# tenpy/tenpy

Hardware: AMD Instinct MI355X
Metric: DMRG sweep time (s) + GS energy err, Heisenberg L=100 chi=2048 (lower is better)
Workload: dtype f64

## Files before the change

include/tenpy_amd.h:

```cpp
#ifndef TENPY_AMD_H
#define TENPY_AMD_H
#include <stdint.h>
#ifdef __cplusplus
extern "C" {
#endif

#define TPA_F64 0
#define TPA_C128 1

#define TPA_E_BADARG (-1)
#define TPA_E_NOCONV (-2)
#define TPA_E_NAN (-3)
#define TPA_E_NOMEM (-4)
#define TPA_E_RANKCAP (-5)

int tpa_version(void);
int tpa_device_info(char *name, int name_len, int *n_cu, int64_t *hbm_bytes);
const char *tpa_last_error(void);

int tpa_gemm_chain(int dtype, int cfg, const int64_t *tasks_dev, const int64_t *links_dev,
                   const int32_t *tiles_dev, int n_tiles, const void *Abase, const void *Bbase,
                   void *Cbase, void *stream);

int tpa_herk_tile_shape(int dtype, int *bt);
int tpa_herk_chain(int dtype, const int64_t *tasks_dev, const int64_t *links_dev, const int32_t *tiles_dev, int n_tiles,
                   const void *Abase, const void *Bbase, const double *wvec_dev, void *Cbase, void *stream);

#define TPA_RED_SCRATCH 4096
int tpa_axpy(int dtype, int64_t n, double alpha_re, double alpha_im, const void *x_dev,
             void *y_dev, void *stream);
int tpa_scal(int dtype, int64_t n, double alpha_re, double alpha_im, void *x_dev, void *stream);
int tpa_dot(int dtype, int64_t n, const void *x_dev, const void *y_dev, int do_conj,
            double *out_dev, double *scratch_dev, void *stream);
int tpa_nrm2sq(int dtype, int64_t n, const void *x_dev, double *out_dev, double *scratch_dev,
               void *stream);
int tpa_lanczos_update(int dtype, int64_t n, void *w_dev, double alpha_re, double alpha_im,
                       const void *v1_dev, double beta_re, double beta_im, const void *v0_dev,
                       double *out_dev, double *scratch_dev, void *stream);
int tpa_lanczos_step(int dtype, int64_t n, void *w_dev, const void *v1_dev, const void *v0_dev,
                     const double *bsq_prev_dev, double *ab_out_dev, double *scratch_dev, void *stream);

#define TPA_PROJECT_MAX 64
#define TPA_PROJECT_WORK (2 * 1024 * (TPA_PROJECT_MAX + 1))
int tpa_project_out(int dtype, int64_t n, const void *basis_dev, int m, int64_t stride, const void *src_dev, void *dst_dev,
                    double *coeff_dev, double *nrm2_out_dev, double *work_dev, void *stream);

typedef int (*tpa_lanczos_callback)(int step, double alpha, double beta_sq, void *user);
typedef int (*tpa_collective_callback)(int which, void *user);
int tpa_lanczos_set_collective(tpa_collective_callback cb, void *user);
int tpa_lanczos_run(int dtype, int64_t n, const int64_t *ops, int n_ops, void *const *bufs, int n_bufs,
                    void *krylov_dev, const void *psi0_dev, int N_max, double cutoff, int has_shift, double E_shift,
                    double *scalars_dev, double *scratch_dev, tpa_lanczos_callback cb, void *user,
                    int time_gemms, double *info, void *stream);
int tpa_lanczos_run_ex(int dtype, int64_t n, const int64_t *ops, int n_ops, void *const *bufs, int n_bufs,
                       void *krylov_dev, const void *psi0_dev, int N_max, double cutoff, int has_shift, double E_shift,
                       double *scalars_dev, double *scratch_dev, tpa_lanczos_callback cb, void *user,
                       int time_gemms, double *info, int flags, double *project_work_dev, void *stream);
int tpa_krylov_combine(int dtype, int64_t n, const void *krylov_dev, int N, const double *coeff, void *out_dev,
                       double *red_out_dev, double *scratch_dev, double *norm_host, void *stream);
int tpa_krylov_combine_z(int basis_dtype, int64_t n, const void *krylov_dev, int N, const double *coeff, double scale,
                         void *out_dev, double *red_out_dev, double *scratch_dev, double *norm_host, void *stream);

#define TPA_COPY_MAXDIM 6
int tpa_copy_batch(int dtype, const int64_t *jobs_dev, int n_jobs, int64_t max_job_elems,
                   const void *src_base, void *dst_base, void *stream);
int tpa_lincomb_batch(int dtype, const int64_t *jobs_dev, int n_jobs, const int64_t *terms_dev, int64_t max_job_elems,
                      const void *src_base, void *dst_base, void *stream);
#define TPA_MPO_APPLY_MAXD 16
int tpa_mpo_apply_batch(int dtype, const int64_t *jobs_dev, int n_jobs, const int64_t *terms_dev, const void *coeff_dev, int max_d,
                        int64_t max_job_elems, const void *src_base, void *dst_base, void *stream);
int tpa_mpo_entry_apply_batch(int dtype, const int64_t *jobs_dev, int n_jobs, const int64_t *rows_dev, const int64_t *terms_dev,
                              int64_t max_job_cols, const void *src_base, void *dst_base, void *stream);
int tpa_scale_axis_batch(int dtype, const int64_t *jobs_dev, int n_jobs, int64_t max_job_elems,
                         void *x_base, const void *s_dev, int s_is_complex, void *stream);
int tpa_fill_zero(void *dst_dev, int64_t n_bytes, void *stream);
int tpa_tri_lower_batch(int dtype, const int64_t *jobs_dev, int n_jobs, int64_t max_job_elems, void *g_base, void *stream);
int tpa_gather_axis_batch(int dtype, const int64_t *jobs_dev, int n_jobs, int64_t max_job_elems,
                          const int64_t *idx_dev, const void *src_base, void *dst_base, void *stream);
int tpa_axis_sqnorm_batch(int dtype, const int64_t *jobs_dev, const int32_t *rows_dev, int n_rows,
                          const void *x_base, double *out_dev, void *stream);
int tpa_convert(int from_dtype, int to_dtype, int64_t n, const void *src_dev, void *dst_dev, int conj,
                void *stream);
int tpa_gemm_tile_shape(int dtype, int cfg, int *bm, int *bn);
int tpa_gemm_set_variant(int v);

int64_t tpa_svd_worksize(int dtype, const int64_t *jobs_host, int n_jobs);
int tpa_svd_batch(int dtype, const int64_t *jobs_host, int n_jobs, const void *a_base,
                  void *u_base, double *s_dev, void *vh_base, void *work_dev, int64_t work_bytes,
                  int max_sweeps, double tol, int *sweeps_done, void *stream);

int tpa_svd_theta(int dtype, int side, const int64_t *blocks, int n_blocks, int64_t a_numel, const void *a_arena,
                  const void *basis_arena, void *u_arena, int64_t u_numel, void *v_arena, int64_t v_numel, double *s_host,
                  double e_tol, int lowdin_basis, int clean_iterations, double clean_floor, int alg_warm, int alg_restore,
                  int max_sweeps, double tol, int *sweeps_done, double *info, void *stream);
int tpa_svd_theta_store(int dtype, const int64_t *blocks, const int64_t *ksig, int n_blocks, const void *u_arena, const void *v_arena,
                        void *basis_r, void *basis_l, void *stream);

int tpa_svd_set_algorithm(int pairwise);
int tpa_svd_dyn_stats(int64_t *out, int reset);
int64_t tpa_svd_call_log(int64_t *out, int64_t max_rows, int reset);
int tpa_svd_set_rank_cap(int cap);

int tpa_qr_batch(int dtype, const int64_t *jobs_host, int n_jobs, const void *a_base, void *q_base,
                 void *r_base, void *stream);
int tpa_qr_set_algorithm(int v);

int64_t tpa_eigh_worksize(int dtype, const int64_t *jobs_host, int n_jobs);
int tpa_eigh_batch(int dtype, const int64_t *jobs_host, int n_jobs, const void *a_base,
                   double *w_dev, void *v_base, void *work_dev, int64_t work_bytes, int max_sweeps,
                   double tol, int *sweeps_done, void *stream);
int tpa_eigh_set_direct(int on);
int tpa_eigh_last_direct(void);
int tpa_eigh_from_svd(int dtype, const int64_t *jobs_host, int n_jobs, const void *u_base, const double *s_dev,
                      const void *vh_base, double *lam_dev, double *err_dev, void *stream);

int tpa_plan_tensordot(const int64_t *a_qdata, int64_t na, int ra, const int64_t *b_qdata,
                       int64_t nb, int rb, int ncontr, const int64_t *contr_nblocks,
                       int64_t *res_qdata, int64_t *res_a_first, int64_t *res_b_first,
                       int64_t cap_res, int64_t *n_res, int64_t *gemm, int64_t cap_gemm,
                       int64_t *n_gemm);

#ifdef __cplusplus
}
#endif
#endif
```

tenpy_amd/_lib.py:

```python
import ctypes
import os

import numpy as np

from . import _build

F64, C128 = 0, 1
E_BADARG, E_NOCONV, E_NAN, E_NOMEM, E_RANKCAP = -1, -2, -3, -4, -5
PROJECT_MAX = 64
PROJECT_WORK = 2 * 1024 * (PROJECT_MAX + 1)
MPO_APPLY_MAXD = 16

_lib = None

_i64p = ctypes.POINTER(ctypes.c_int64)
_vp = ctypes.c_void_p
LANCZOS_CALLBACK = ctypes.CFUNCTYPE(ctypes.c_int, ctypes.c_int, ctypes.c_double, ctypes.c_double, ctypes.c_void_p)
COLLECTIVE_CALLBACK = ctypes.CFUNCTYPE(ctypes.c_int, ctypes.c_int, ctypes.c_void_p)
_SIGS = {
    "tpa_version": (ctypes.c_int, []),
    "tpa_last_error": (ctypes.c_char_p, []),
    "tpa_device_info": (ctypes.c_int, [ctypes.c_char_p, ctypes.c_int, ctypes.POINTER(ctypes.c_int), _i64p]),
    "tpa_gemm_tile_shape": (ctypes.c_int, [ctypes.c_int, ctypes.c_int, ctypes.POINTER(ctypes.c_int), ctypes.POINTER(ctypes.c_int)]),
    "tpa_gemm_set_variant": (ctypes.c_int, [ctypes.c_int]),
    "tpa_gemm_chain": (ctypes.c_int, [ctypes.c_int, ctypes.c_int, _vp, _vp, _vp, ctypes.c_int, _vp, _vp, _vp, _vp]),
    "tpa_herk_tile_shape": (ctypes.c_int, [ctypes.c_int, ctypes.POINTER(ctypes.c_int)]),
    "tpa_herk_chain": (ctypes.c_int, [ctypes.c_int, _vp, _vp, _vp, ctypes.c_int, _vp, _vp, _vp, _vp, _vp]),
    "tpa_axpy": (ctypes.c_int, [ctypes.c_int, ctypes.c_int64, ctypes.c_double, ctypes.c_double, _vp, _vp, _vp]),
    "tpa_scal": (ctypes.c_int, [ctypes.c_int, ctypes.c_int64, ctypes.c_double, ctypes.c_double, _vp, _vp]),
    "tpa_dot": (ctypes.c_int, [ctypes.c_int, ctypes.c_int64, _vp, _vp, ctypes.c_int, _vp, _vp, _vp]),
    "tpa_nrm2sq": (ctypes.c_int, [ctypes.c_int, ctypes.c_int64, _vp, _vp, _vp, _vp]),
    "tpa_lanczos_update": (ctypes.c_int, [ctypes.c_int, ctypes.c_int64, _vp, ctypes.c_double, ctypes.c_double, _vp,
                                          ctypes.c_double, ctypes.c_double, _vp, _vp, _vp, _vp]),
    "tpa_lanczos_step": (ctypes.c_int, [ctypes.c_int, ctypes.c_int64, _vp, _vp, _vp, _vp, _vp, _vp, _vp]),
    "tpa_lanczos_run": (ctypes.c_int, [ctypes.c_int, ctypes.c_int64, _vp, ctypes.c_int, _vp, ctypes.c_int, _vp, _vp, ctypes.c_int,
                                       ctypes.c_double, ctypes.c_int, ctypes.c_double, _vp, _vp, _vp, _vp, ctypes.c_int, _vp, _vp]),
    "tpa_lanczos_run_ex": (ctypes.c_int, [ctypes.c_int, ctypes.c_int64, _vp, ctypes.c_int, _vp, ctypes.c_int, _vp, _vp, ctypes.c_int,
                                          ctypes.c_double, ctypes.c_int, ctypes.c_double, _vp, _vp, _vp, _vp, ctypes.c_int, _vp,
                                          ctypes.c_int, _vp, _vp]),
    "tpa_project_out": (ctypes.c_int, [ctypes.c_int, ctypes.c_int64, _vp, ctypes.c_int, ctypes.c_int64, _vp, _vp, _vp, _vp, _vp, _vp]),
    "tpa_lanczos_set_collective": (ctypes.c_int, [COLLECTIVE_CALLBACK, _vp]),
    "tpa_krylov_combine": (ctypes.c_int, [ctypes.c_int, ctypes.c_int64, _vp, ctypes.c_int, _vp, _vp, _vp, _vp, _vp, _vp]),
    "tpa_krylov_combine_z": (ctypes.c_int, [ctypes.c_int, ctypes.c_int64, _vp, ctypes.c_int, _vp, ctypes.c_double, _vp, _vp, _vp, _vp, _vp]),
    "tpa_copy_batch": (ctypes.c_int, [ctypes.c_int, _vp, ctypes.c_int, ctypes.c_int64, _vp, _vp, _vp]),
    "tpa_lincomb_batch": (ctypes.c_int, [ctypes.c_int, _vp, ctypes.c_int, _vp, ctypes.c_int64, _vp, _vp, _vp]),
    "tpa_mpo_apply_batch": (ctypes.c_int, [ctypes.c_int, _vp, ctypes.c_int, _vp, _vp, ctypes.c_int, ctypes.c_int64, _vp, _vp, _vp]),
    "tpa_mpo_entry_apply_batch": (ctypes.c_int, [ctypes.c_int, _vp, ctypes.c_int, _vp, _vp, ctypes.c_int64, _vp, _vp, _vp]),
    "tpa_svd_dyn_stats": (ctypes.c_int, [_i64p, ctypes.c_int]),
    "tpa_tri_lower_batch": (ctypes.c_int, [ctypes.c_int, _vp, ctypes.c_int, ctypes.c_int64, _vp, _vp]),
    "tpa_scale_axis_batch": (ctypes.c_int, [ctypes.c_int, _vp, ctypes.c_int, ctypes.c_int64, _vp, _vp, ctypes.c_int, _vp]),
    "tpa_gather_axis_batch": (ctypes.c_int, [ctypes.c_int, _vp, ctypes.c_int, ctypes.c_int64, _vp, _vp, _vp, _vp]),
    "tpa_axis_sqnorm_batch": (ctypes.c_int, [ctypes.c_int, _vp, _vp, ctypes.c_int, _vp, _vp, _vp]),
    "tpa_convert": (ctypes.c_int, [ctypes.c_int, ctypes.c_int, ctypes.c_int64, _vp, _vp, ctypes.c_int, _vp]),
    "tpa_fill_zero": (ctypes.c_int, [_vp, ctypes.c_int64, _vp]),
    "tpa_svd_worksize": (ctypes.c_int64, [ctypes.c_int, _vp, ctypes.c_int]),
    "tpa_svd_batch": (ctypes.c_int, [ctypes.c_int, _vp, ctypes.c_int, _vp, _vp, _vp, _vp, _vp, ctypes.c_int64,
                                     ctypes.c_int, ctypes.c_double, ctypes.POINTER(ctypes.c_int), _vp]),
    "tpa_svd_set_algorithm": (ctypes.c_int, [ctypes.c_int]),
    "tpa_svd_theta": (ctypes.c_int, [ctypes.c_int, ctypes.c_int, _vp, ctypes.c_int, ctypes.c_int64, _vp, _vp, _vp, ctypes.c_int64, _vp, ctypes.c_int64,
                                     _vp, ctypes.c_double, ctypes.c_int, ctypes.c_int, ctypes.c_double, ctypes.c_int, ctypes.c_int, ctypes.c_int,
                                     ctypes.c_double, ctypes.POINTER(ctypes.c_int), _vp, _vp]),
    "tpa_svd_theta_store": (ctypes.c_int, [ctypes.c_int, _vp, _vp, ctypes.c_int, _vp, _vp, _vp, _vp, _vp]),
    "tpa_svd_set_rank_cap": (ctypes.c_int, [ctypes.c_int]),
    "tpa_svd_call_log": (ctypes.c_int64, [_i64p, ctypes.c_int64, ctypes.c_int]),
    "tpa_qr_batch": (ctypes.c_int, [ctypes.c_int, _vp, ctypes.c_int, _vp, _vp, _vp, _vp]),
    "tpa_qr_set_algorithm": (ctypes.c_int, [ctypes.c_int]),
    "tpa_eigh_worksize": (ctypes.c_int64, [ctypes.c_int, _vp, ctypes.c_int]),
    "tpa_eigh_batch": (ctypes.c_int, [ctypes.c_int, _vp, ctypes.c_int, _vp, _vp, _vp, _vp, ctypes.c_int64,
                                      ctypes.c_int, ctypes.c_double, ctypes.POINTER(ctypes.c_int), _vp]),
    "tpa_eigh_set_direct": (ctypes.c_int, [ctypes.c_int]),
    "tpa_eigh_last_direct": (ctypes.c_int, []),
    "tpa_eigh_from_svd": (ctypes.c_int, [ctypes.c_int, _vp, ctypes.c_int, _vp, _vp, _vp, _vp, _vp, _vp]),
    "tpa_plan_tensordot": (ctypes.c_int, [_vp, ctypes.c_int64, ctypes.c_int, _vp, ctypes.c_int64, ctypes.c_int,
                                          ctypes.c_int, _vp, _vp, _vp, _vp, ctypes.c_int64, _i64p, _vp,
                                          ctypes.c_int64, _i64p]),
}


class BackendError(RuntimeError):
    """The HIP extension is missing or a HIP runtime call failed."""


def load(build_if_missing=True):
    global _lib
    if _lib is not None:
        return _lib
    import torch
    path = _build.LIB_PATH
    alt = os.environ.get('TPA_LIB_PATH')
    if alt:
        if not os.path.exists(alt):
            raise BackendError("tenpy_amd: TPA_LIB_PATH=%s does not exist" % alt)
        path, build_if_missing = alt, False
    if not os.path.exists(path):
        if not build_if_missing:
            raise BackendError("tenpy_amd: %s not built; run `python -m tenpy_amd._build`" % path)
        _build.build()
    elif build_if_missing and os.path.exists(_build.HIPCC) and os.path.isdir(_build.CSRC) and not os.environ.get('TPA_NO_AUTOBUILD'):
        import fcntl
        try:
            with open(os.path.join(_build.OUT_DIR, '.build.lock'), 'w') as lock:
                fcntl.flock(lock, fcntl.LOCK_EX)
                try:
                    _build.build()
                finally:
                    fcntl.flock(lock, fcntl.LOCK_UN)
        except OSError:
            pass
    lib = ctypes.CDLL(path)
    for name, (res, args) in _SIGS.items():
        f = getattr(lib, name)
        f.restype = res
        f.argtypes = args
    _lib = lib
    return lib


def exported_symbols():
    return sorted(_SIGS)


def check(rc, what=""):
    if rc == 0:
        return
    msg = load().tpa_last_error()
    msg = msg.decode() if msg else ""
    if rc == E_BADARG:
        raise ValueError("tenpy_amd %s: %s" % (what, msg))
    if rc == E_NOCONV:
        raise np.linalg.LinAlgError("tenpy_amd %s: %s" % (what, msg))
    if rc == E_NAN:
        raise ValueError("tenpy_amd %s: NaN/Inf encountered: %s" % (what, msg))
    raise BackendError("tenpy_amd %s: HIP error %d: %s" % (what, rc, msg))


_gpu_ok = False


def require_gpu():
    global _gpu_ok
    if _gpu_ok:
        return
    import torch
    if not torch.cuda.is_available():
        raise BackendError("tenpy_amd: no GPU visible (torch.cuda.is_available() is False); "
                           "this backend has no CPU fallback")
    load()
    _gpu_ok = True
```

tenpy_amd/algorithms/mps_common.py:

```python
import numpy as np

from ..linalg import _device as dev
from ..linalg import np_conserved as npc

__all__ = ['TwoSiteH', 'OneSiteH', 'ZeroSiteH']


FUSED_HEFF = True
import os as _os
FACTORED_MATVEC = _os.environ.get('TPA_FACTORED_MATVEC', '1') != '0'
FACTORED_MIN_SECTOR = 200
BLOCK_APPLY = _os.environ.get('TPA_MPO_BLOCK_APPLY', '1') != '0'
from .._lib import MPO_APPLY_MAXD
ENTRY_APPLY = int(_os.environ.get('TPA_MPO_ENTRY_APPLY', '1'))

def _env_set_LP(env, i, LP):
    if hasattr(env, 'get_LP_age'):
        env.set_LP(i, LP, age=(env.get_LP_age(i - 1) or 0) + 1)
    else:
        env.set_LP(i, LP)


def _env_set_RP(env, i, RP):
    if hasattr(env, 'get_RP_age'):
        env.set_RP(i, RP, age=(env.get_RP_age(i + 1) or 0) + 1)
    else:
        env.set_RP(i, RP)


def _mpo_entries(W):
    ent = getattr(W, '_tpa_entries', False)
    if ent is False:
        if all(np.all(leg.get_block_sizes() == 1) for leg in W.legs) and W.stored_blocks > 0:
            vals = np.array([np.asarray(b).reshape(-1)[0] for b in W._data])
            ent = (np.array(W._qdata), vals)
        else:
            ent = None
        W._tpa_entries = ent
    return ent


def _mpo_blocks(W):
    blk = getattr(W, '_tpa_blocks', False)
    if blk is False:
        labels = list(W.get_leg_labels())
        blk = None
        if W.rank == 4 and 'wL' in labels and 'wR' in labels and W.stored_blocks > 0 and W.chinfo.qnumber > 0:
            phys = [a for a in range(4) if labels[a] not in ('wL', 'wR')]
            if all(np.all(W.get_leg(l).get_block_sizes() == 1) for l in ('wL', 'wR')) and \
                    all(int(np.max(W.legs[a].get_block_sizes())) <= MPO_APPLY_MAXD for a in phys):
                blk = (np.array(W._qdata), [np.array(b) for b in W._data])
        W._tpa_blocks = blk
    return blk


def _share_mpo_tables(W_new, W):
    W_new._tpa_entries = _mpo_entries(W)
    if W_new._tpa_entries is None and BLOCK_APPLY and dev.lib_provides('tpa_mpo_apply_batch'):
        W_new._tpa_blocks = _mpo_blocks(W)
    W_new._tpa_origin = W


def _mpo_coo(W):
    coo = getattr(W, '_tpa_coo', False)
    if coo is False and getattr(W, '_tpa_origin', None) is not None:
        coo = W._tpa_coo = _mpo_coo(W._tpa_origin)
    if coo is False:
        labels = list(W.get_leg_labels())
        coo = None
        if W.rank == 4 and 'wL' in labels and 'wR' in labels and W.stored_blocks > 0:
            idx, vals = [], []
            for q, b in zip(np.array(W._qdata).tolist(), W._data):
                b = np.array(b)
                nz = np.nonzero(b)
                idx.append(np.stack([nz[a] + int(W.legs[a].slices[q[a]]) for a in range(4)], axis=1))
                vals.append(b[nz])
            coo = (np.concatenate(idx).astype(np.int64).reshape(-1, 4), np.concatenate(vals))
        W._tpa_coo = coo
    return coo


def _pack_alpha(terms, alpha):
    alpha = np.asarray(alpha, dtype=np.complex128)
    terms[:, 2] = np.ascontiguousarray(alpha.real).view(np.int64)
    terms[:, 3] = np.ascontiguousarray(alpha.imag).view(np.int64)


def _lincomb_into(dst, src, jobs, terms, max_elems):
    if len(jobs) == 0:
        return
    L = dev.lib()
    terms_d = dev.table(terms)
    for s0 in range(0, len(jobs), 60000):
        jd = dev.table(jobs[s0:s0 + 60000])
        dev.check(L.tpa_lincomb_batch(dev.code(dst.dtype), jd.data_ptr(), len(jobs[s0:s0 + 60000]), terms_d.data_ptr(),
                                      int(max_elems), src._arena.data_ptr(), dst._arena.data_ptr(), dev.stream()), "lincomb")


def _rank_rows(q):
    uq, inv = np.unique(q, axis=0, return_inverse=True)
    order = np.lexsort(uq.T)
    rank_of = np.empty(len(order), dtype=np.int64)
    rank_of[order] = np.arange(len(order))
    return uq[order], rank_of[inv.reshape(-1)]


def _group_terms(dst):
    key = np.lexsort((np.arange(len(dst)), dst))
    d_sorted = dst[key]
    starts = np.nonzero(np.concatenate([[True], d_sorted[1:] != d_sorted[:-1]]))[0]
    return key, starts, np.diff(np.concatenate([starts, [len(key)]]))


from collections import OrderedDict as _OrderedDict
_heff_plans = _OrderedDict()


def _fused_heff(env_t, W, left):
    from ..linalg.charges import LegPipe
    ent = _mpo_entries(W)
    pl = 'p0' if left else 'p1'
    want_env = ['vR*', 'wR', 'vR'] if left else ['wL', 'vL', 'vL*']
    if ent is None or list(env_t.get_leg_labels()) != want_env or list(W.get_leg_labels()) != ['wL', 'wR', pl, pl + '*'] \
            or env_t.dtype != np.result_type(env_t.dtype, W.dtype) or env_t.stored_blocks == 0:
        return None
    wq, wv = ent
    w_axis_env = 1 if left else 0
    if not np.all(env_t.legs[w_axis_env].get_block_sizes() == 1):
        return None
    pkey = (left, env_t._struct_key(), env_t.dtype.str, id(ent), env_t.qtotal.tobytes(),
            tuple((l.charges.tobytes(), int(l.qconj)) for l in env_t.legs))
    plan = _heff_plans.get(pkey)
    if plan is not None and plan['ent'] is ent:
        try:
            _heff_plans.move_to_end(pkey)
        except KeyError:
            pass
        res = npc.Array(plan['legs'], env_t.dtype, plan['qtotal'], plan['labels'])
        res._adopt_blocks(plan['qdata'], plan['offsets'], dev.zeros(plan['total'], env_t.dtype), True)
        dev.check(dev.lib().tpa_lincomb_batch(dev.code(env_t.dtype), plan['jobs'].data_ptr(), plan['n_jobs'], plan['terms'].data_ptr(),
                                              plan['max_elems'], env_t._arena.data_ptr(), res._arena.data_ptr(), dev.stream()), "lincomb")
        return res, plan['pipe']
    eq = env_t._qdata
    shapes = env_t._block_shapes()
    if left:
        pipe = LegPipe([env_t.get_leg('vR*'), W.get_leg('p0')], qconj=+1)
        legs = [pipe, W.get_leg('wR'), pipe.conj()]
        labels = ['(vR*.p0)', 'wR', '(vR.p0*)']
    else:
        pipe = LegPipe([W.get_leg('p1'), env_t.get_leg('vL*')], qconj=-1)
        legs = [W.get_leg('wL'), pipe.conj(), pipe]
        labels = ['wL', '(p1*.vL)', '(p1.vL*)']
    qm = pipe.q_map
    n0, n1 = pipe.legs[0].block_number, pipe.legs[1].block_number
    row_of = np.full((n0, n1), -1, dtype=np.int64)
    row_of[qm[:, 3], qm[:, 4]] = np.arange(len(qm))
    psz = pipe.get_block_sizes()
    wc = wq[:, 0] if left else wq[:, 1]
    ie, iw = np.nonzero(eq[:, w_axis_env][:, None] == wc[None, :])
    if len(ie) == 0:
        return None
    if left:
        r_row = row_of[eq[ie, 0], wq[iw, 2]]
        c_row = row_of[eq[ie, 2], wq[iw, 3]]
        w_out = wq[iw, 1]
        rows, cols = shapes[ie, 0], shapes[ie, 2]
    else:
        r_row = row_of[wq[iw, 3], eq[ie, 1]]
        c_row = row_of[wq[iw, 2], eq[ie, 2]]
        w_out = wq[iw, 0]
        rows, cols = shapes[ie, 1], shapes[ie, 2]
    Qr, Qc = qm[r_row, 2], qm[c_row, 2]
    r0, c0 = qm[r_row, 0], qm[c_row, 0]
    bq = np.stack([Qr, w_out, Qc], axis=1) if left else np.stack([w_out, Qr, Qc], axis=1)
    ubq, blk = _rank_rows(bq)
    res = npc.Array(legs, env_t.dtype, env_t.chinfo.make_valid(env_t.qtotal + W.qtotal), labels)
    res._set_blocks(ubq, zero=True, qdata_sorted=True)
    ld = psz[Qc]
    dst_off = res._offsets[blk] + r0 * ld + c0
    perm, starts, counts = _group_terms(dst_off)
    jobs = np.zeros((len(starts), 8), dtype=np.int64)
    pf = perm[starts]
    jobs[:, 0], jobs[:, 1], jobs[:, 2], jobs[:, 3] = dst_off[pf], rows[pf], cols[pf], ld[pf]
    jobs[:, 4], jobs[:, 5] = starts, counts
    terms = np.zeros((len(perm), 4), dtype=np.int64)
    terms[:, 0] = env_t._offsets[ie[perm]]
    terms[:, 1] = shapes[ie[perm], 2]
    _pack_alpha(terms, wv[iw[perm]])
    _lincomb_into(res, env_t, jobs, terms, int(np.max(rows * cols)))
    if 0 < len(jobs) <= 60000:
        for arr in (res._qdata, res._offsets):
            arr.setflags(write=False)
        _heff_plans[pkey] = dict(ent=ent, legs=legs, labels=labels, qtotal=res.qtotal.copy(), qdata=res._qdata, offsets=res._offsets,
                                 total=int(res._arena.numel()), jobs=dev.table(jobs), terms=dev.table(terms), n_jobs=len(jobs),
                                 max_elems=int(np.max(rows * cols)), pipe=pipe)
        if len(_heff_plans) > 8192:
            _heff_plans.popitem(last=False)
    return res, pipe


def _reverse_columns(U):
    res = npc.Array(U.legs, U.dtype, U.qtotal, list(U._labels))
    res._set_blocks(U._qdata, zero=False, qdata_sorted=U._qdata_sorted)
    if U.stored_blocks == 0:
        return res
    shapes = U._block_shapes()
    m, k = shapes[:, 0], shapes[:, 1]
    blk = np.repeat(np.arange(len(k)), k)
    col = np.arange(len(blk)) - np.repeat(np.cumsum(k) - k, k)
    jobs = np.zeros((len(blk), 8), dtype=np.int64)
    jobs[:, 0] = res._offsets[blk] + col
    jobs[:, 1], jobs[:, 2], jobs[:, 3] = m[blk], 1, k[blk]
    jobs[:, 4], jobs[:, 5] = np.arange(len(blk)), 1
    terms = np.zeros((len(blk), 4), dtype=np.int64)
    terms[:, 0] = U._offsets[blk] + (k[blk] - 1 - col)
    terms[:, 1] = k[blk]
    terms[:, 2] = np.array([1.0]).view(np.int64)[0]
    _lincomb_into(res, U, jobs, terms, int(np.max(m)))
    return res


def _relabel_view(A, labels):
    perm = [A.get_leg_index(l) for l in labels]
    if perm == list(range(A.rank)):
        return A
    big = [a for a in range(A.rank) if not np.all(A.legs[a].get_block_sizes() == 1)]
    assert [a for a in perm if a in big] == big, "only legs with 1-wide blocks may be moved"
    B = A.copy(deep=False)
    B.legs = [A.legs[a] for a in perm]
    B._set_shape()
    B._labels = [A._labels[a] for a in perm]
    B._qdata = np.ascontiguousarray(A._qdata[:, perm])
    B._offsets = A._offsets.copy()
    B._qdata_sorted = False
    B._skey = None
    B.isort_qdata()
    return B


class _MpoStepPlan:

    @classmethod
    def get(cls, X, W, *args, W2=None, **kwargs):
        t1, t2 = cls._table(W), (None if W2 is None else cls._table(W2))
        key = (X._struct_key(), str(X.dtype), id(t1), None if t2 is None else id(t2), args,
               tuple(sorted(kwargs.items())), tuple(X.get_leg_labels()))
        plan = cls._cache.get(key)
        if plan is None or plan._tables_alive[0] is not t1 or plan._tables_alive[1] is not t2:
            if len(cls._cache) > 4096:
                cls._cache.clear()
            plan = cls._cache[key] = cls(X, W, *args, W2=W2, **kwargs)
            plan._tables_alive = (t1, t2)
        return plan

    @staticmethod
    def _match_blocks(X, keys, xa):
        xq = X._qdata
        match = xq[:, xa[0]][:, None] == keys[None, :, 0]
        for a, col in zip(xa[1:], (3, 5)):
            match &= xq[:, a][:, None] == keys[None, :, col]
        ib, ie = np.nonzero(match)
        oq = xq[ib].copy()
        for a, col in zip(xa, (1, 2, 4)):
            oq[:, a] = keys[ie, col]
        return ib, ie, oq

    def _set_output(self, X, W, W2, xa, w_out, p_out, p2_out, out_labels):
        self.dtype = np.result_type(X.dtype, W.dtype) if W2 is None else np.result_type(X.dtype, W.dtype, W2.dtype)
# ... 294 lines not shown
        self.x_key = X._struct_key()
        self.bytes = 8 * (2 if self.dtype.kind == 'c' else 1) * (self.total + int(np.sum(shapes_x[ib, 0] * post_x)))

    def _launch(self, X, res):
        dev.check(dev.lib().tpa_mpo_entry_apply_batch(dev.code(self.dtype), self.jobs_dev.data_ptr(), self.n_jobs, self.rows_dev.data_ptr(),
                                                      self.terms_dev.data_ptr(), self.max_cols, X._arena.data_ptr(), res._arena.data_ptr(),
                                                      dev.stream()), "mpo_entry_apply")

    def program_op(self, a_slot, c_slot):
        return [6, 0, self.jobs_dev.data_ptr(), self.rows_dev.data_ptr(), self.terms_dev.data_ptr(), self.n_jobs, a_slot, 0, c_slot,
                self.max_cols, 0, 0]


def _envs_wide(LP, RP):
    return not (bool(np.all(LP.get_leg('wR').get_block_sizes() == 1)) and bool(np.all(RP.get_leg('wL').get_block_sizes() == 1)))


def _envs_factorable(LP, RP):
    lp, rp = list(LP.get_leg_labels()), list(RP.get_leg_labels())
    return (sorted(lp) == sorted(['vR*', 'wR', 'vR']) and lp.index('vR*') < lp.index('vR') and
            sorted(rp) == sorted(['wL', 'vL', 'vL*']) and rp.index('vL') < rp.index('vL*') and
            (not _envs_wide(LP, RP) or _entry_route(LP.chinfo)))


def _env_form(A, labels):
    if list(A.get_leg_labels()) == list(labels):
        return A
    w = 'wR' if 'wR' in labels else 'wL'
    if np.all(A.get_leg(w).get_block_sizes() == 1):
        return _relabel_view(A, labels)
    return A.transpose(labels)


def _factored_plan_class(LP, RP, W, W2=None):
    if not _envs_factorable(LP, RP):
        return None
    cls = _mpo_plan_class(W, W2)
    if cls is not MpoEntryApplyPlan and _envs_wide(LP, RP):
        return None
    return cls


def factored_matvec_possible(LP, RP, W0, W1):
    w0, w1 = list(W0.get_leg_labels()), list(W1.get_leg_labels())
    return (_factored_plan_class(LP, RP, W0, W1) is not None and
            w0 in (['wL', 'wR', 'p0', 'p0*'], ['wL', 'wR', 'p', 'p*']) and w1 in (['wL', 'wR', 'p1', 'p1*'], ['wL', 'wR', 'p', 'p*']))


def _gemm_ops(plan, a_slot, b_slot, c_slot, bufs, scratch_name):
    sk = plan.sk
    if sk is None:
        return [[0, plan.cfg, plan.tasks_dev.data_ptr(), plan.links_dev.data_ptr(), plan.tiles_dev.data_ptr(), plan.n_tiles,
                 a_slot, b_slot, c_slot, 0, 0, 0]]
    bufs.append(dev.scratch(scratch_name, sk.total, plan.dtype))
    part = len(bufs) - 1
    return [[0, plan.cfg, sk.tasks_dev.data_ptr(), sk.links_dev.data_ptr(), sk.tiles_dev.data_ptr(), sk.n_tiles, a_slot, b_slot, part, 0, 0, 0],
            [1, 1, sk.jobs_dev.data_ptr(), sk.terms_dev.data_ptr(), 0, sk.n_jobs, part, 0, c_slot, sk.max_elems, 0, 0]]


_STEP_LR = ('wR', 'p0', 'wL', 'wR', 'p0', 'p0*')
_STEP_RL = ('wL', 'p1', 'wR', 'wL', 'p1', 'p1*')


def _mpo_step_lr(X, W0, W1=None, *, out_labels):
    two = {} if W1 is None else dict(W2=W1, x_p2='p1', p2_out='p1', p2_in='p1*')
    return _mpo_plan_class(W0, W1).get(X, W0, *_STEP_LR, tuple(out_labels), **two)


def _mpo_step_rl(X, W1, *, out_labels):
    return _mpo_plan_class(W1).get(X, W1, *_STEP_RL, tuple(out_labels))


def _factored_plans(LPf, RPf, theta, W0, W1=None, launch=False, old=None):
    keys = dict(key=theta._struct_key(), dtype=theta.dtype, lkey=LPf._struct_key(), rkey=RPf._struct_key())
    if old is not None and all(old[k] == v for k, v in keys.items()):
        return old, None, None
    p1, l_use, t_use = npc.plan_tensordot(LPf, theta, axes=['vR', 'vL'])
    fits = l_use is LPf and t_use is theta
    assert fits or not launch, "factored matvec step 1 must not need a transpose"
    if not fits or (p1.empty and not launch):
        return None, None, None
    T = T1 = p1.apply(LPf, theta, launch=launch)
    a = None
    if W0 is not None:
        a = _mpo_step_lr(T1, W0, W1, out_labels=('vR*', 'p0', 'wR', 'vR') if W1 is None else ('vR*', 'p0', 'p1', 'wR', 'vR'))
        if a.empty and not launch:
            return None, None, None
        T = a.apply(T1, launch=launch)
    p2, t_use, r_use = npc.plan_tensordot(T, RPf, axes=(['wR', 'vR'], ['wL', 'vL']))
    fits = t_use is T and r_use is RPf
    assert fits or not launch, "factored matvec step 2 must not need a transpose"
    if not fits or (p2.empty and not launch):
        return None, None, None
    return dict(keys, p1=p1, p2=p2, **{'a0' if W1 is None else 'a01': a}), T1, T


class _DeviceEffectiveH:

    def _file_program(self, theta, res, last):
        key = (theta._struct_key(), theta.dtype)
        self.__dict__['_program_out'] = None
        if res is not None and not (last.res_total == theta._arena.numel() and np.array_equal(last.res_qdata, theta._qdata)
                                    and np.array_equal(last.res_offsets, theta._offsets)):
            self.__dict__['_program_out'] = (key, last.res_qdata, last.res_offsets, last.res_total)
            res = None
        self.__dict__['_program'] = (key, res)
        return res

    def native_input(self, theta, max_pad=2):
        vec = theta
        for _ in range(max_pad + 1):
            prog = self.matvec_program(vec)
            if prog is not None:
                return vec, prog
            out = self.__dict__.get('_program_out')
            if out is None or out[0] != (vec._struct_key(), vec.dtype):
                return None
            _, qdata, offsets, total = out
            have = {tuple(r) for r in qdata.tolist()}
            if not all(tuple(r) in have for r in vec._qdata.tolist()):
                return None
            pad = npc.Array(vec.legs, vec.dtype, vec.qtotal, vec.get_leg_labels())
            pad._set_blocks(qdata, arena=dev.zeros(total, vec.dtype), qdata_sorted=True)
            if not np.array_equal(pad._offsets, offsets):
                return None
            npc._scatter_blocks(vec, pad, pad._arena)
            vec = pad
        return None


class TwoSiteH(_DeviceEffectiveH):
    length = 2
    acts_on = ['(vL.p0)', '(p1.vR)']

    def __init__(self, env, i0, combine=True, move_right=True, tensors=None, factored=None):
        if not combine:
            raise NotImplementedError("tenpy_amd.TwoSiteH (stand-alone driver): only combine=True")
        self.i0 = i0
        self.combine = combine
        self.move_right = move_right
        if tensors is not None:
            self.LP, self.RP, W0, W1 = tensors
            self.dtype = W0.dtype
        else:
            self.LP = env.get_LP(i0)
            self.RP = env.get_RP(i0 + 1)
            W0, W1 = env.H.get_W(i0), env.H.get_W(i0 + 1)
            self.dtype = env.H.dtype
        self.W0 = W0.replace_labels(['p', 'p*'], ['p0', 'p0*'])
        self.W1 = W1.replace_labels(['p', 'p*'], ['p1', 'p1*'])
        _share_mpo_tables(self.W0, W0)
        _share_mpo_tables(self.W1, W1)
        self._env = env
        self._LHeff = self._RHeff = None
        self._plans = None
        self._fplans = None
        if factored is None:
            want = FACTORED_MATVEC and int(np.max(self.LP.get_leg('vR').get_block_sizes())) >= FACTORED_MIN_SECTOR
        else:
            want = factored
        self.factored = bool(want) and self._factored_possible()
        if self.factored:
            from ..linalg.charges import LegPipe
            self._LPf = _env_form(self.LP, ['vR*', 'wR', 'vR'])
            self._RPf = _env_form(self.RP, ['wL', 'vL', 'vL*'])
            self.pipeL = LegPipe([self.LP.get_leg('vR*'), self.W0.get_leg('p0')], qconj=+1)
            self.pipeR = LegPipe([self.W1.get_leg('p1'), self.RP.get_leg('vL*')], qconj=-1)
            self._LHeff = self._RHeff = None
            self.acts_on = ['vL', 'p0', 'p1', 'vR']
        else:
            self.combine_Heff(self._env)
        self.N = self.pipeL.ind_len * self.pipeR.ind_len
        self.flops_per_matvec = None
        self.bytes_per_matvec = None

    def _factored_possible(self):
        return factored_matvec_possible(self.LP, self.RP, self.W0, self.W1)

    @property
    def LHeff(self):
        if self._LHeff is None:
            self._build_heff_lazily()
        return self._LHeff

    @LHeff.setter
    def LHeff(self, value):
        self._LHeff = value

    @property
    def RHeff(self):
        if self._RHeff is None:
            self._build_heff_lazily()
        return self._RHeff

    @RHeff.setter
    def RHeff(self, value):
        self._RHeff = value

    def _build_heff_lazily(self):
        pL, pR = self.pipeL, self.pipeR
        self.combine_Heff(self._env)
        pL.test_equal(self.pipeL)
        pR.test_equal(self.pipeR)
        self.pipeL, self.pipeR = pL, pR

    def combine_Heff(self, env=None):
        cache = getattr(env, '_heff_cache', None) if env is not None else None
        hit = cache.get(('L', self.i0)) if cache is not None else None
        if hit is not None and hit[0] is self.LP:
            _, self.LHeff, self.pipeL = hit
        else:
            fused = _fused_heff(self.LP, self.W0, True) if FUSED_HEFF else None
            if fused is not None:
                self.LHeff, self.pipeL = fused
            else:
                LHeff = npc.tensordot(self.LP, self.W0, axes=['wR', 'wL'])
                self.pipeL = pipeL = LHeff.make_pipe(['vR*', 'p0'], qconj=+1)
                self.LHeff = LHeff.combine_legs([['vR*', 'p0'], ['vR', 'p0*']], pipes=[pipeL, pipeL.conj()],
                                                new_axes=[0, 2])
            if cache is not None:
                cache[('L', self.i0)] = (self.LP, self.LHeff, self.pipeL)
        hit = cache.get(('R', self.i0 + 1)) if cache is not None else None
        if hit is not None and hit[0] is self.RP:
            _, self.RHeff, self.pipeR = hit
        else:
            fused = _fused_heff(self.RP, self.W1, False) if FUSED_HEFF else None
            if fused is not None:
                self.RHeff, self.pipeR = fused
            else:
                RHeff = npc.tensordot(self.W1, self.RP, axes=['wR', 'wL'])
                self.pipeR = pipeR = RHeff.make_pipe(['p1', 'vL*'], qconj=-1)
                self.RHeff = RHeff.combine_legs([['p1*', 'vL'], ['p1', 'vL*']], pipes=[pipeR.conj(), pipeR],
                                                new_axes=[1, 2])
            if cache is not None:
                cache[('R', self.i0 + 1)] = (self.RP, self.RHeff, self.pipeR)

    def combine_theta(self, theta):
        if self.factored:
            if theta.rank == 2:
                theta = theta.split_legs()
            return theta if list(theta.get_leg_labels()) == ['vL', 'p0', 'p1', 'vR'] else theta.transpose(['vL', 'p0', 'p1', 'vR'])
        return theta.combine_legs([['vL', 'p0'], ['p1', 'vR']], pipes=[self.pipeL, self.pipeR])

    def prepare_svd(self, theta):
        if theta.rank == 2:
            return theta
        return theta.combine_legs([['vL', 'p0'], ['p1', 'vR']], pipes=[self.pipeL, self.pipeR])

    def _matvec_factored(self, theta):
        fp, T3 = self._plans_for(theta, launch=True)
        if T3 is None:
            T3 = fp['a01'].apply(fp['p1'].apply(self._LPf, theta))
        res = fp['p2'].apply(T3, self._RPf)
        res.iset_leg_labels(['vL', 'p0', 'p1', 'vR'])
        return res

    def _plans_for(self, theta, launch):
        fp, _, T3 = _factored_plans(self._LPf, self._RPf, theta, self.W0, self.W1, launch, old=self._fplans)
        if fp is not None and fp is not self._fplans:
            self._fplans = fp
            p1, p2 = fp['p1'], fp['p2']
            if not p1.empty and not p2.empty:
                self.flops_per_matvec = p1.flops + p2.flops
                self.bytes_per_matvec = p1.bytes_min + p2.bytes_min + fp['a01'].bytes
                self.gemm_shapes = (p1.gemm_shapes, p2.gemm_shapes)
        return fp, T3

    def matvec(self, theta):
        if self.factored:
            if theta.rank == 2:
                return self.prepare_svd(self._matvec_factored(self.combine_theta(theta)))
            return self._matvec_factored(theta)
        if self._plans is None or not self._plan_matches(theta):
            p1, l_use, t_use = npc.plan_tensordot(self.LHeff, theta, axes=['(vR.p0*)', '(vL.p0)'])
            assert l_use is self.LHeff and t_use is theta, "matvec step 1 must not need a transpose"
            tmp = p1.apply(self.LHeff, theta)
            p2, t2_use, r_use = npc.plan_tensordot(tmp, self.RHeff, axes=(['wR', '(p1.vR)'], ['wL', '(p1*.vL)']))
            assert t2_use is tmp and r_use is self.RHeff, "matvec step 2 must not need a transpose"
            self._plans = (p1, p2, theta._struct_key(), theta.dtype)
            if not p1.empty and not p2.empty:
                self.flops_per_matvec = p1.flops + p2.flops
                self.bytes_per_matvec = p1.bytes_min + p2.bytes_min
                self.gemm_shapes = (p1.gemm_shapes, p2.gemm_shapes)
            res = p2.apply(tmp, self.RHeff)
        else:
            p1, p2 = self._plans[0], self._plans[1]
            tmp = p1.apply(self.LHeff, theta)
            res = p2.apply(tmp, self.RHeff)
        res.iset_leg_labels(['(vL.p0)', '(p1.vR)'])
        return res

    def matvec_program(self, theta):
        want = ['vL', 'p0', 'p1', 'vR'] if self.factored else ['(vL.p0)', '(p1.vR)']
        if list(theta.get_leg_labels()) != want or theta.stored_blocks == 0 or not theta._is_packed():
            return None
        key = (theta._struct_key(), theta.dtype)
        prog = self.__dict__.get('_program')
        if prog is not None and prog[0] == key:
            return prog[1]
        res = None
        if self.factored:
            fp = self._plans_for(theta, launch=False)[0]
            if fp is None:
                return None
            p1, a01, p2 = fp['p1'], fp['a01'], fp['p2']
            ok = (p1.dtype == a01.dtype == p2.dtype == theta.dtype == self._LPf.dtype == self._RPf.dtype and not p1.empty and
                  not p2.empty and not a01.empty)
            if ok:
                bufs = [self._LPf._arena, self._RPf._arena, dev.scratch('lanczos_t1', p1.res_total, p1.dtype),
                        dev.scratch('lanczos_t3', a01.total, a01.dtype)]
                ops = _gemm_ops(p1, 0, -1, 2, bufs, 'lanczos_sk1')
                ops.append(a01.program_op(2, 3))
                ops += _gemm_ops(p2, 3, 1, -2, bufs, 'lanczos_sk2')
                res = (np.array(ops, dtype=np.int64), bufs, (p1, p2))
                last = p2
        else:
            if self._plans is None or not self._plan_matches(theta):
                p1, l_use, t_use = npc.plan_tensordot(self.LHeff, theta, axes=['(vR.p0*)', '(vL.p0)'])
                if l_use is not self.LHeff or t_use is not theta or p1.empty:
                    return None
                tmp = p1.apply(self.LHeff, theta, launch=False)
                p2, t2_use, r_use = npc.plan_tensordot(tmp, self.RHeff, axes=(['wR', '(p1.vR)'], ['wL', '(p1*.vL)']))
                if t2_use is not tmp or r_use is not self.RHeff or p2.empty:
                    return None
                self._plans = (p1, p2, theta._struct_key(), theta.dtype)
                self.flops_per_matvec = p1.flops + p2.flops
                self.bytes_per_matvec = p1.bytes_min + p2.bytes_min
                self.gemm_shapes = (p1.gemm_shapes, p2.gemm_shapes)
            p1, p2 = self._plans[0], self._plans[1]
            if p1.dtype == p2.dtype == theta.dtype == self.LHeff.dtype == self.RHeff.dtype and not p1.empty and not p2.empty:
                bufs = [self.LHeff._arena, self.RHeff._arena, dev.scratch('lanczos_t1', p1.res_total, p1.dtype)]
                ops = _gemm_ops(p1, 0, -1, 2, bufs, 'lanczos_sk1') + _gemm_ops(p2, 2, 1, -2, bufs, 'lanczos_sk2')
                res = (np.array(ops, dtype=np.int64), bufs, (p1, p2))
                last = p2
        return self._file_program(theta, res, last if res is not None else None)

    def _plan_matches(self, theta):
        return self._plans[2] == theta._struct_key() and self._plans[3] == theta.dtype

    def update_LP(self, env, i, U=None):
        assert i == self.i0 + 1
        if self.factored:
            A = U.split_legs(['(vL.p0)'])
            cls = _mpo_plan_class(self.W0)
            X = npc.tensordot(self._LPf if cls is MpoEntryApplyPlan else self.LP, A, axes=['vR', 'vL'])
            X = _mpo_step_lr(X, self.W0, out_labels=('vR*', 'p0', 'wR', 'vR')).apply(X)
            LP = npc.tensordot(A.conj(), X, axes=(['vL*', 'p0*'], ['vR*', 'p0']))
            LP = _env_form(LP, list(self.LP.get_leg_labels()))
            _env_set_LP(env, i, LP)
            return LP
        LP = npc.tensordot(self.LHeff, U, axes=['(vR.p0*)', '(vL.p0)'])
        LP = npc.tensordot(U.conj(), LP, axes=['(vL*.p0*)', '(vR*.p0)'])
        _env_set_LP(env, i, LP)
        return LP

    def update_RP(self, env, i, VH=None):
        assert i == self.i0
        if self.factored:
            B = VH.split_legs(['(p1.vR)'])
            cls = _mpo_plan_class(self.W1)
            X = npc.tensordot(B, self._RPf if cls is MpoEntryApplyPlan else self.RP, axes=['vR', 'vL'])
            X = _mpo_step_rl(X, self.W1, out_labels=('vL', 'wL', 'p1', 'vL*')).apply(X)
            RP = npc.tensordot(X, B.conj(), axes=(['p1', 'vL*'], ['p1*', 'vR*']))
            RP = _env_form(RP, list(self.RP.get_leg_labels()))
            _env_set_RP(env, i, RP)
            return RP
        RP = npc.tensordot(VH, self.RHeff, axes=['(p1.vR)', '(p1*.vL)'])
        RP = npc.tensordot(RP, VH.conj(), axes=['(p1.vL*)', '(p1*.vR*)'])
        _env_set_RP(env, i, RP)
        return RP

    def adjoint(self):
        return AdjointH(self)

    def plus_hc(self):
        return _plus_hc_operator(self)

    def to_matrix_array(self):
        contr = npc.tensordot(self.LHeff, self.RHeff, axes=['wR', 'wL'])
        return contr.combine_legs([['(vR*.p0)', '(p1.vL*)'], ['(vR.p0*)', '(p1*.vL)']], qconj=[+1, -1])

    def to_matrix(self):
        L, R = self.LHeff.to_ndarray(), self.RHeff.to_ndarray()
        full = np.tensordot(L, R, axes=([1], [0]))
        full = full.transpose(0, 3, 1, 2)
        n = full.shape[0] * full.shape[1]
        return full.reshape(n, n)


class _LocalH(_DeviceEffectiveH):
    combine = False
    move_right = True
    _env = None

    def _setup(self, LP, W0, RP, i0, dtype):
        self.i0 = i0
        self.LP, self.RP = LP, RP
        self.W0 = None
        if W0 is not None:
            self.W0 = W0.replace_labels(['p', 'p*'], ['p0', 'p0*'])
            _share_mpo_tables(self.W0, W0)
        self.dtype = dtype
        self._fplans = None
        if W0 is None:
            self.factored = _envs_factorable(LP, RP)
        else:
            self.factored = (list(self.W0.get_leg_labels()) == ['wL', 'wR', 'p0', 'p0*'] and
                             _factored_plan_class(LP, RP, self.W0) is not None)
        if self.factored:
            self._LPf = _env_form(LP, ['vR*', 'wR', 'vR'])
            self._RPf = _env_form(RP, ['wL', 'vL', 'vL*'])
        n = LP.get_leg('vR').ind_len * RP.get_leg('vL').ind_len
        self.N = n if W0 is None else n * self.W0.get_leg('p0').ind_len

    def _plans(self, theta):
        self._fplans = _factored_plans(self._LPf, self._RPf, theta, self.W0, old=self._fplans)[0]
        return self._fplans

    def matvec(self, theta):
        labels = list(theta.get_leg_labels())
        if labels != self.acts_on:
            theta = theta.transpose(self.acts_on)
        fp = self._plans(theta) if (self.factored and theta.stored_blocks > 0) else None
        if fp is not None:
            T = fp['p1'].apply(self._LPf, theta)
            if fp['a0'] is not None:
                T = fp['a0'].apply(T)
            res = fp['p2'].apply(T, self._RPf)
        else:
            res = npc.tensordot(self.LP, theta, axes=['vR', 'vL'])
            if self.W0 is not None:
                res = npc.tensordot(self.W0, res, axes=[['wL', 'p0*'], ['wR', 'p0']])
            res = npc.tensordot(res, self.RP, axes=[['wR', 'vR'], ['wL', 'vL']])
            res = res.replace_labels(['vR*', 'vL*'], ['vL', 'vR']).transpose(self.acts_on)
        res.iset_leg_labels(self.acts_on)
        return res if labels == self.acts_on else res.transpose(labels)

    def matvec_program(self, theta):
        if not self.factored or list(theta.get_leg_labels()) != self.acts_on or theta.stored_blocks == 0 or not theta._is_packed():
            return None
        key = (theta._struct_key(), theta.dtype)
        prog = self.__dict__.get('_program')
        if prog is not None and prog[0] == key:
            return prog[1]
        fp = self._plans(theta)
        res = last = None
        if fp is not None:
            p1, a0, p2 = fp['p1'], fp['a0'], fp['p2']
            if p1.dtype == p2.dtype == theta.dtype == self._LPf.dtype == self._RPf.dtype and (a0 is None or a0.dtype == theta.dtype):
                bufs = [self._LPf._arena, self._RPf._arena, dev.scratch('lanczos_t1', p1.res_total, p1.dtype)]
                ops = _gemm_ops(p1, 0, -1, 2, bufs, 'lanczos_sk1')
                src = 2
                if a0 is not None:
                    bufs.append(dev.scratch('lanczos_t3', a0.total, a0.dtype))
                    src = len(bufs) - 1
                    ops.append(a0.program_op(2, src))
                ops += _gemm_ops(p2, src, 1, -2, bufs, 'lanczos_sk2')
                res, last = (np.array(ops, dtype=np.int64), bufs, (p1, p2)), p2
        return self._file_program(theta, res, last)

    def adjoint(self):
        return AdjointH(self)

    def plus_hc(self):
        return _plus_hc_operator(self)

    def to_matrix(self):
        contr = self.LP
        if self.W0 is not None:
            contr = npc.tensordot(contr, self.W0, axes=['wR', 'wL'])
        contr = npc.tensordot(contr, self.RP, axes=['wR', 'wL'])
        if self.W0 is not None:
            return contr.combine_legs([['vR*', 'p0', 'vL*'], ['vR', 'p0*', 'vL']], qconj=[+1, -1])
        return contr.combine_legs([['vR*', 'vL*'], ['vR', 'vL']], qconj=[+1, -1])


class OneSiteH(_LocalH):
    length = 1
    acts_on = ['vL', 'p0', 'vR']

    def __init__(self, env, i0, combine=False, move_right=True):
        if combine:
            raise NotImplementedError("tenpy_amd.OneSiteH (stand-alone driver): only combine=False")
        self.move_right = move_right
        self._env = env
        self._setup(env.get_LP(i0), env.H.get_W(i0), env.get_RP(i0), i0, env.H.dtype)

    @classmethod
    def from_LP_W0_RP(cls, LP, W0, RP, i0=0, combine=False, move_right=True):
        if combine:
            raise NotImplementedError("tenpy_amd.OneSiteH: only combine=False")
# ... 258 lines not shown
```

tenpy_amd/csrc/tpa_gemm.hip:

```cpp
#include "tpa_common.h"

typedef double d4 __attribute__((ext_vector_type(4)));

namespace {

struct Link {
    int64_t a_off, b_off, k, a_rs, a_ks, b_ks, b_ns, flags;
};
struct Task {
    int64_t c_off, m, n, ldc, link_begin, link_count, accumulate, pad;
};

template <int ES, int NT, int BM, int BN>
__device__ __forceinline__ bool gemm_identity_rows_tile(const Task &tk, const Link *__restrict__ links, const int4 tile, const double *__restrict__ Bbase,
                                                        double *__restrict__ Cbase, const int tid) {
    if (tile.w <= 0 || tk.pad == 0) return false;
    if (reinterpret_cast<const int *>(tk.pad)[tile.w - 1] != 0) return false;
    const Link L = links[tk.link_begin];
    const int row0 = tile.y * BM, col0 = tile.z * BN;
    const int rows = min(BM, (int)tk.m - row0), cols = min(BN, (int)tk.n - col0);
    for (int e = tid; e < rows * BN; e += NT) {
        const int r = e / BN, c = e % BN;
        if (c < cols) {
            const int64_t src = L.b_off + (int64_t)(row0 + r) * L.b_ks + (int64_t)(col0 + c) * L.b_ns;
            const int64_t dst = tk.c_off + (int64_t)(row0 + r) * tk.ldc + col0 + c;
#pragma unroll
            for (int q = 0; q < ES; ++q) Cbase[ES * dst + q] = Bbase[ES * src + q];
        }
    }
    return true;
}

template <bool CPLX, int BM, int BN, int TM, int TN, int BK_>
struct Cfg {
    static constexpr int BK = BK_;
    static constexpr int WM = BM / (TM * 16);
    static constexpr int WN = BN / (TN * 16);
    static constexpr int NT = WM * WN * 64;
    static constexpr int PADA = 16, PADB = 16;
    static constexpr int A_LDS = (BM * (BK + 1) > BK * (BM + PADA)) ? BM * (BK + 1) : BK * (BM + PADA);
    static constexpr int B_LDS = (BN * (BK + 1) > BK * (BN + PADB)) ? BN * (BK + 1) : BK * (BN + PADB);
    static constexpr int PLANES = CPLX ? 2 : 1;
    static constexpr int EA = BM * BK / NT;
    static constexpr int EB = BN * BK / NT;
    static_assert(NT % BK == 0 && NT % BM == 0 && NT % BN == 0, "staging offsets must be affine in the element index");
};

struct Stage {
    const double *p;
    int64_t gstep, kstep;
    int lbase, lstep, kk0, kkstep;
    int i0, istep, lim;
};

template <bool CPLX, int BM, int BN, int TM, int TN, int BK_>
__global__ __launch_bounds__((Cfg<CPLX, BM, BN, TM, TN, BK_>::NT)) void gemm_chain_kernel(
    const Task *__restrict__ tasks, const Link *__restrict__ links, const int4 *__restrict__ tiles,
    const double *__restrict__ Abase, const double *__restrict__ Bbase, double *__restrict__ Cbase) {
    using C = Cfg<CPLX, BM, BN, TM, TN, BK_>;
    constexpr int NT = C::NT, EA = C::EA, EB = C::EB, PL = C::PLANES, BK = C::BK;
    constexpr int ES = CPLX ? 2 : 1;
    __shared__ double lds[PL * (C::A_LDS + C::B_LDS)];
    double *As = lds;
    double *Bs = lds + PL * C::A_LDS;

    const int4 tile = tiles[blockIdx.x];
    const Task tk = tasks[tile.x];
    const int m = (int)tk.m, n = (int)tk.n;
    const int row0 = tile.y * BM, col0 = tile.z * BN;
    const int tid = threadIdx.x, lane = tid & 63, wave = tid >> 6;
    const int wr = wave / C::WN, wc = wave % C::WN;
    const int l15 = lane & 15, l4 = lane >> 4;
    if (gemm_identity_rows_tile<ES, NT, BM, BN>(tk, links, tile, Bbase, Cbase, tid)) return;

    d4 acc[PL][TM][TN];
#pragma unroll
    for (int p = 0; p < PL; ++p)
#pragma unroll
        for (int i = 0; i < TM; ++i)
#pragma unroll
            for (int j = 0; j < TN; ++j) acc[p][i][j] = d4{0, 0, 0, 0};

    const int nl = (int)tk.link_count;
    const Link *lk = links + tk.link_begin;

    struct LinkView {
        Stage a, b;
        int K, sa_i, sa_k, sb_j, sb_k;
        double sgn_a, sgn_b;
        int64_t oa[EA], ob[EB];
    };
    auto open_link = [&](int li, LinkView &v) {
        const Link L = lk[li];
        v.K = (int)L.k;
        const bool a_kfast = (L.a_ks == 1);
        const bool b_kfast = (L.b_ks == 1) && (L.b_ns != 1);
        v.sgn_a = (CPLX && (L.flags & 1)) ? -1.0 : 1.0;
        v.sgn_b = (CPLX && (L.flags & 2)) ? -1.0 : 1.0;
        v.sa_i = a_kfast ? (BK + 1) : 1;
        v.sa_k = a_kfast ? 1 : (BM + C::PADA);
        v.sb_j = b_kfast ? (BK + 1) : 1;
        v.sb_k = b_kfast ? 1 : (BN + C::PADB);
        {
            const int i = a_kfast ? (tid / BK) : (tid % BM), kk = a_kfast ? (tid % BK) : (tid / BM);
            const int di = a_kfast ? (NT / BK) : 0, dk = a_kfast ? 0 : (NT / BM);
            v.a.p = Abase + ES * (L.a_off + (int64_t)(row0 + i) * L.a_rs + (int64_t)kk * L.a_ks);
            v.a.gstep = ES * ((int64_t)di * L.a_rs + (int64_t)dk * L.a_ks);
            v.a.kstep = ES * (int64_t)BK * L.a_ks;
            v.a.lbase = i * v.sa_i + kk * v.sa_k;
            v.a.lstep = di * v.sa_i + dk * v.sa_k;
            v.a.kk0 = kk;
            v.a.kkstep = dk;
            v.a.i0 = row0 + i;
            v.a.istep = di;
            v.a.lim = m;
#pragma unroll
            for (int r = 0; r < EA; ++r) v.oa[r] = r * v.a.gstep;
        }
        {
            const int j = b_kfast ? (tid / BK) : (tid % BN), kk = b_kfast ? (tid % BK) : (tid / BN);
            const int dj = b_kfast ? (NT / BK) : 0, dk = b_kfast ? 0 : (NT / BN);
            v.b.p = Bbase + ES * (L.b_off + (int64_t)kk * L.b_ks + (int64_t)(col0 + j) * L.b_ns);
            v.b.gstep = ES * ((int64_t)dk * L.b_ks + (int64_t)dj * L.b_ns);
            v.b.kstep = ES * (int64_t)BK * L.b_ks;
            v.b.lbase = kk * v.sb_k + j * v.sb_j;
            v.b.lstep = dk * v.sb_k + dj * v.sb_j;
            v.b.kk0 = kk;
            v.b.kkstep = dk;
            v.b.i0 = col0 + j;
            v.b.istep = dj;
            v.b.lim = n;
#pragma unroll
            for (int r = 0; r < EB; ++r) v.ob[r] = r * v.b.gstep;
        }
    };
    double ra[PL][EA], rb[PL][EB];
    auto load_tile = [&](LinkView &v, int k0) {
        const int krem = v.K - k0;
        const bool full = (krem >= BK);
#pragma unroll
        for (int r = 0; r < EA; ++r) {
            const bool ok = (v.a.i0 + r * v.a.istep < v.a.lim) && (full || v.a.kk0 + r * v.a.kkstep < krem);
            const double *q = v.a.p + v.oa[r];
            if (CPLX) {
                double2 x = ok ? *reinterpret_cast<const double2 *>(q) : double2{0, 0};
                ra[0][r] = x.x;
                ra[PL - 1][r] = v.sgn_a * x.y;
            } else {
                ra[0][r] = ok ? *q : 0.0;
            }
        }
#pragma unroll
        for (int r = 0; r < EB; ++r) {
            const bool ok = (v.b.i0 + r * v.b.istep < v.b.lim) && (full || v.b.kk0 + r * v.b.kkstep < krem);
            const double *q = v.b.p + v.ob[r];
            if (CPLX) {
                double2 x = ok ? *reinterpret_cast<const double2 *>(q) : double2{0, 0};
                rb[0][r] = x.x;
                rb[PL - 1][r] = v.sgn_b * x.y;
            } else {
                rb[0][r] = ok ? *q : 0.0;
            }
        }
        v.a.p += v.a.kstep;
        v.b.p += v.b.kstep;
    };

    auto store_tile = [&](const LinkView &v, double *Ad, double *Bd) {
#pragma unroll
        for (int r = 0; r < EA; ++r)
#pragma unroll
            for (int p = 0; p < PL; ++p) Ad[p * C::A_LDS + v.a.lbase + r * v.a.lstep] = ra[p][r];
#pragma unroll
        for (int r = 0; r < EB; ++r)
#pragma unroll
            for (int p = 0; p < PL; ++p) Bd[p * C::B_LDS + v.b.lbase + r * v.b.lstep] = rb[p][r];
    };
    auto mma_tile = [&](const double *Aw, const double *Bw, int sa_i, int sa_k, int sb_j, int sb_k) {
#pragma unroll
        for (int ks = 0; ks < BK / 4; ++ks) {
            double a[PL][TM], b[PL][TN];
#pragma unroll
            for (int p = 0; p < PL; ++p) {
#pragma unroll
                for (int i = 0; i < TM; ++i) a[p][i] = Aw[p * C::A_LDS + i * 16 * sa_i + ks * 4 * sa_k];
#pragma unroll
                for (int j = 0; j < TN; ++j) b[p][j] = Bw[p * C::B_LDS + j * 16 * sb_j + ks * 4 * sb_k];
            }
#pragma unroll
            for (int i = 0; i < TM; ++i)
#pragma unroll
                for (int j = 0; j < TN; ++j) {
                    if (CPLX) {
                        acc[0][i][j] = __builtin_amdgcn_mfma_f64_16x16x4f64(a[0][i], b[0][j], acc[0][i][j], 0, 0, 0);
                        acc[0][i][j] = __builtin_amdgcn_mfma_f64_16x16x4f64(-a[PL - 1][i], b[PL - 1][j], acc[0][i][j], 0, 0, 0);
                        acc[PL - 1][i][j] = __builtin_amdgcn_mfma_f64_16x16x4f64(a[0][i], b[PL - 1][j], acc[PL - 1][i][j], 0, 0, 0);
                        acc[PL - 1][i][j] = __builtin_amdgcn_mfma_f64_16x16x4f64(a[PL - 1][i], b[0][j], acc[PL - 1][i][j], 0, 0, 0);
                    } else {
                        acc[0][i][j] = __builtin_amdgcn_mfma_f64_16x16x4f64(a[0][i], b[0][j], acc[0][i][j], 0, 0, 0);
                    }
                }
        }
    };

    int li = 0;
    while (li < nl && lk[li].k <= 0) ++li;
    if (li < nl) {
        LinkView cur, nxt;
        open_link(li, cur);
        load_tile(cur, 0);
        while (true) {
            int lj = li + 1;
            while (lj < nl && lk[lj].k <= 0) ++lj;
            const bool has_next = lj < nl;
            if (has_next) open_link(lj, nxt);
            const int K = cur.K;
            const int sa_i = cur.sa_i, sa_k = cur.sa_k, sb_j = cur.sb_j, sb_k = cur.sb_k;
            const int fa = (wr * TM * 16 + l15) * sa_i + l4 * sa_k, fb = (wc * TN * 16 + l15) * sb_j + l4 * sb_k;
            for (int k0 = 0; k0 < K; k0 += BK) {
                store_tile(cur, As, Bs);
                __syncthreads();
                if (k0 + BK < K)
                    load_tile(cur, k0 + BK);
                else if (has_next)
                    load_tile(nxt, 0);
                mma_tile(As + fa, Bs + fb, sa_i, sa_k, sb_j, sb_k);
                __syncthreads();
            }
            if (!has_next) break;
            cur = nxt;
            li = lj;
        }
    }

    double *Cp = Cbase + ES * tk.c_off;
    const bool accum = tk.accumulate != 0;
#pragma unroll
    for (int i = 0; i < TM; ++i)
#pragma unroll
        for (int j = 0; j < TN; ++j)
#pragma unroll
            for (int r = 0; r < 4; ++r) {
                const int row = row0 + wr * TM * 16 + i * 16 + l4 + 4 * r;
                const int col = col0 + wc * TN * 16 + j * 16 + l15;
                if (row < m && col < n) {
                    const int64_t g = (int64_t)row * tk.ldc + col;
                    if (CPLX) {
                        double2 v{acc[0][i][j][r], acc[PL - 1][i][j][r]};
                        double2 *dst = reinterpret_cast<double2 *>(Cp + 2 * g);
                        if (accum) {
                            double2 o = *dst;
                            v.x += o.x;
                            v.y += o.y;
                        }
                        *dst = v;
                    } else {
                        double v = acc[0][i][j][r];
                        if (accum) v += Cp[g];
                        Cp[g] = v;
                    }
                }
            }
}


template <int BM, int BN, int TM, int TN>
struct Cfg2 {
    static constexpr int BK = 16, LD = BK + 1;
    static constexpr int WM = BM / (TM * 16), WN = BN / (TN * 16), NT = WM * WN * 64;
    static constexpr int A_LDS = BM * LD, B_LDS = BN * LD, IMG = A_LDS + B_LDS;
    static constexpr int EA = BM * BK / NT, EB = BN * BK / NT;
    static constexpr int LDS_BYTES = 2 * IMG * 8;
    static_assert(NT % BK == 0 && NT % BM == 0 && NT % BN == 0, "staging offsets must be affine in the element index");
};

template <int BM, int BN, int TM, int TN>
__global__ __launch_bounds__((Cfg2<BM, BN, TM, TN>::NT)) __attribute__((amdgpu_waves_per_eu(TM * TN >= 16 ? 2 : (TM * TN >= 8 ? 3 : 4))))
void gemm_chain2_kernel(
    const Task *__restrict__ tasks, const Link *__restrict__ links, const int4 *__restrict__ tiles,
    const double *__restrict__ Abase, const double *__restrict__ Bbase, double *__restrict__ Cbase) {
    using C = Cfg2<BM, BN, TM, TN>;
    constexpr int NT = C::NT, EA = C::EA, EB = C::EB, BK = C::BK, LD = C::LD, IMG = C::IMG;
    extern __shared__ double lds2[];

    const int4 tile = tiles[blockIdx.x];
    const Task tk = tasks[tile.x];
    const int m = (int)tk.m, n = (int)tk.n;
    const int row0 = tile.y * BM, col0 = tile.z * BN;
    const int tid = threadIdx.x, lane = tid & 63, wave = __builtin_amdgcn_readfirstlane(tid >> 6);
    const int wr = wave / C::WN, wc = wave % C::WN;
    const int l15 = lane & 15, l4 = lane >> 4;
    const bool wave_act = (row0 + wr * TM * 16 < m) && (col0 + wc * TN * 16 < n);
    if (gemm_identity_rows_tile<1, NT, BM, BN>(tk, links, tile, Bbase, Cbase, tid)) return;

    d4 acc[TM][TN];
#pragma unroll
    for (int i = 0; i < TM; ++i)
#pragma unroll
        for (int j = 0; j < TN; ++j) acc[i][j] = d4{0, 0, 0, 0};

    const int nl = (int)tk.link_count;
    const Link *lk = links + tk.link_begin;

    struct View {
        const double *pa, *pb;
        int64_t ka, kb;
        int64_t oa[EA], ob[EB];
        int kka, dka, kkb, dkb;
        int la, dla, lb, dlb;
        int K;
    };
    auto open_link = [&](int li, View &v) {
        const Link L = lk[li];
        v.K = (int)L.k;
        const bool a_kfast = (L.a_ks == 1);
        const bool b_kfast = (L.b_ks == 1) && (L.b_ns != 1);
        {
            const int i = a_kfast ? (tid / BK) : (tid % BM), kk = a_kfast ? (tid % BK) : (tid / BM);
            const int di = a_kfast ? (NT / BK) : 0, dk = a_kfast ? 0 : (NT / BM);
            v.pa = Abase + L.a_off;
            v.ka = (int64_t)BK * L.a_ks;
            v.kka = kk;
            v.dka = dk;
            v.la = i * LD + kk;
            v.dla = di * LD + dk;
#pragma unroll
            for (int r = 0; r < EA; ++r)
                v.oa[r] = (int64_t)min(row0 + i + r * di, m - 1) * L.a_rs + (int64_t)(kk + r * dk) * L.a_ks;
        }
        {
            const int j = b_kfast ? (tid / BK) : (tid % BN), kk = b_kfast ? (tid % BK) : (tid / BN);
            const int dj = b_kfast ? (NT / BK) : 0, dk = b_kfast ? 0 : (NT / BN);
            v.pb = Bbase + L.b_off;
            v.kb = (int64_t)BK * L.b_ks;
            v.kkb = kk;
            v.dkb = dk;
            v.lb = j * LD + kk;
            v.dlb = dj * LD + dk;
#pragma unroll
            for (int r = 0; r < EB; ++r)
                v.ob[r] = (int64_t)min(col0 + j + r * dj, n - 1) * L.b_ns + (int64_t)(kk + r * dk) * L.b_ks;
        }
    };
    double ra[EA], rb[EB];
    auto load_tile = [&](View &v, int krem) {
        if (krem >= BK) {
#pragma unroll
            for (int r = 0; r < EA; ++r) ra[r] = v.pa[v.oa[r]];
#pragma unroll
            for (int r = 0; r < EB; ++r) rb[r] = v.pb[v.ob[r]];
        } else {
#pragma unroll
            for (int r = 0; r < EA; ++r) ra[r] = (v.kka + r * v.dka < krem) ? v.pa[v.oa[r]] : 0.0;
#pragma unroll
            for (int r = 0; r < EB; ++r) rb[r] = (v.kkb + r * v.dkb < krem) ? v.pb[v.ob[r]] : 0.0;
        }
        v.pa += v.ka;
        v.pb += v.kb;
    };
    auto store_tile = [&](const View &v, double *img) {
#pragma unroll
        for (int r = 0; r < EA; ++r) img[v.la + r * v.dla] = ra[r];
#pragma unroll
        for (int r = 0; r < EB; ++r) img[C::A_LDS + v.lb + r * v.dlb] = rb[r];
    };
    const int fa0 = (wr * TM * 16 + l15) * LD + l4, fb0 = C::A_LDS + (wc * TN * 16 + l15) * LD + l4;
    double fa[2][TM], fb[2][TN];
    auto read_frag = [&](const double *img, int ks, int buf) {
#pragma unroll
        for (int i = 0; i < TM; ++i) fa[buf][i] = img[fa0 + i * 16 * LD + ks * 4];
#pragma unroll
        for (int j = 0; j < TN; ++j) fb[buf][j] = img[fb0 + j * 16 * LD + ks * 4];
    };
    auto mma_step = [&](int buf) {
        if (wave_act) {
#pragma unroll
            for (int i = 0; i < TM; ++i)
#pragma unroll
                for (int j = 0; j < TN; ++j)
                    acc[i][j] = __builtin_amdgcn_mfma_f64_16x16x4f64(fa[buf][i], fb[buf][j], acc[i][j], 0, 0, 0);
        }
    };

    View st;
    int li = 0;
    while (li < nl && lk[li].k <= 0) ++li;
    if (li < nl) {
        open_link(li, st);
        int kdone = 0;
        auto load_next = [&]() -> bool {
            if (kdone >= st.K) {
                int lj = li + 1;
                while (lj < nl && lk[lj].k <= 0) ++lj;
                if (lj >= nl) return false;
                li = lj;
                open_link(li, st);
                kdone = 0;
            }
            load_tile(st, st.K - kdone);
            kdone += BK;
            return true;
        };
        load_next();
        store_tile(st, lds2);
        bool have = load_next();
        lds_barrier();
        int img = 0;
        while (true) {
            const double *cur = lds2 + img * IMG;
            double *oth = lds2 + (img ^ 1) * IMG;
            read_frag(cur, 0, 0);
            read_frag(cur, 1, 1);
            mma_step(0);
            const bool had = have;
            if (had) {
                store_tile(st, oth);
                have = load_next();
            }
            read_frag(cur, 2, 0);
            mma_step(1);
            read_frag(cur, 3, 1);
            mma_step(0);
            mma_step(1);
            if (!had) break;
            lds_barrier();
            img ^= 1;
        }
    }

    double *Cp = Cbase + tk.c_off;
    const bool accum = tk.accumulate != 0;
#pragma unroll
    for (int i = 0; i < TM; ++i)
#pragma unroll
        for (int j = 0; j < TN; ++j)
#pragma unroll
            for (int r = 0; r < 4; ++r) {
                const int row = row0 + wr * TM * 16 + i * 16 + l4 + 4 * r;
                const int col = col0 + wc * TN * 16 + j * 16 + l15;
                if (row < m && col < n) {
                    const int64_t g = (int64_t)row * tk.ldc + col;
                    double v = acc[i][j][r];
                    if (accum) v += Cp[g];
                    Cp[g] = v;
                }
            }
}

}

#include <stdlib.h>
static int g_variant = getenv("TPA_GEMM_VARIANT") ? atoi(getenv("TPA_GEMM_VARIANT")) : 0;

extern "C" int tpa_gemm_set_variant(int v) {
    g_variant = v;
    return 0;
}

extern "C" int tpa_gemm_tile_shape(int dtype, int cfg, int *bm, int *bn) {
    *bm = cfg ? 64 : 128;
    *bn = (dtype == TPA_F64) ? 64 : (cfg ? 32 : 64);
    return 0;
}

template <bool CPLX, int BM, int BN, int TM, int TN, int BK_>
static void launch(const int64_t *tasks_dev, const int64_t *links_dev, const int32_t *tiles_dev, int n_tiles,
                   const void *Abase, const void *Bbase, void *Cbase, hipStream_t st) {
    using C = Cfg<CPLX, BM, BN, TM, TN, BK_>;
    gemm_chain_kernel<CPLX, BM, BN, TM, TN, BK_><<<n_tiles, C::NT, 0, st>>>(
        (const Task *)tasks_dev, (const Link *)links_dev, (const int4 *)tiles_dev, (const double *)Abase,
        (const double *)Bbase, (double *)Cbase);
}

template <int BM, int BN, int TM, int TN>
static int launch2(const int64_t *tasks_dev, const int64_t *links_dev, const int32_t *tiles_dev, int n_tiles,
                   const void *Abase, const void *Bbase, void *Cbase, hipStream_t st) {
    using C = Cfg2<BM, BN, TM, TN>;
    static bool attr_set = false;
    if (!attr_set) {
        TPA_HIP_CHECK(hipFuncSetAttribute((const void *)gemm_chain2_kernel<BM, BN, TM, TN>, hipFuncAttributeMaxDynamicSharedMemorySize,
                                          C::LDS_BYTES));
        attr_set = true;
    }
    gemm_chain2_kernel<BM, BN, TM, TN><<<n_tiles, C::NT, C::LDS_BYTES, st>>>(
        (const Task *)tasks_dev, (const Link *)links_dev, (const int4 *)tiles_dev, (const double *)Abase,
        (const double *)Bbase, (double *)Cbase);
    return 0;
}

extern "C" int tpa_gemm_chain(int dtype, int cfg, const int64_t *tasks_dev, const int64_t *links_dev,
                              const int32_t *tiles_dev, int n_tiles, const void *Abase,
                              const void *Bbase, void *Cbase, void *stream) {
    TPA_ARG_CHECK(dtype == TPA_F64 || dtype == TPA_C128);
    TPA_ARG_CHECK(cfg == 0 || cfg == 1);
    if (n_tiles <= 0) return 0;
    hipStream_t st = (hipStream_t)stream;
    int rc = 0;
    if (dtype == TPA_F64) {
        if (cfg == 0)
            rc = launch2<128, 64, 4, 2>(tasks_dev, links_dev, tiles_dev, n_tiles, Abase, Bbase, Cbase, st);
        else if (n_tiles <= 1024 && !(g_variant & 1))
            launch<false, 64, 64, 1, 2, 16>(tasks_dev, links_dev, tiles_dev, n_tiles, Abase, Bbase, Cbase, st);
        else
            rc = launch2<64, 64, 2, 2>(tasks_dev, links_dev, tiles_dev, n_tiles, Abase, Bbase, Cbase, st);
    } else {
        if (cfg == 1)
            launch<true, 64, 32, 2, 1, 16>(tasks_dev, links_dev, tiles_dev, n_tiles, Abase, Bbase, Cbase, st);
        else
            launch<true, 128, 64, 4, 2, 16>(tasks_dev, links_dev, tiles_dev, n_tiles, Abase, Bbase, Cbase, st);
    }
    if (rc) return rc;
    TPA_LAUNCH_CHECK();
    return 0;
}
```

tenpy_amd/csrc/tpa_util.hip:

```cpp
#include "tpa_common.h"
#include <string.h>

extern "C" int tpa_device_info(char *name, int name_len, int *n_cu, int64_t *hbm_bytes) {
    int dev = 0;
    TPA_HIP_CHECK(hipGetDevice(&dev));
    hipDeviceProp_t p;
    TPA_HIP_CHECK(hipGetDeviceProperties(&p, dev));
    if (name && name_len > 0) {
        strncpy(name, p.gcnArchName, (size_t)name_len - 1);
        name[name_len - 1] = 0;
    }
    if (n_cu) *n_cu = p.multiProcessorCount;
    if (hbm_bytes) *hbm_bytes = (int64_t)p.totalGlobalMem;
    return 0;
}
```

tenpy_amd/csrc/tpa_vec.hip:

```cpp
#include "tpa_common.h"
#include <vector>

namespace {

constexpr int NT = 256;
constexpr int MAXBLK = 1024;

__host__ inline int grid_for(int64_t n, int per_thread) {
    int64_t g = (n + (int64_t)NT * per_thread - 1) / ((int64_t)NT * per_thread);
    if (g < 1) g = 1;
    if (g > MAXBLK) g = MAXBLK;
    return (int)g;
}

__global__ __launch_bounds__(NT) void axpy_f64(int64_t n, double a, const double *__restrict__ x,
                                               double *__restrict__ y) {
    for (int64_t i = (int64_t)blockIdx.x * NT + threadIdx.x; i < n; i += (int64_t)gridDim.x * NT)
        y[i] = fma(a, x[i], y[i]);
}
__global__ __launch_bounds__(NT) void axpy_c128(int64_t n, double ar, double ai,
                                                const double2 *__restrict__ x,
                                                double2 *__restrict__ y) {
    for (int64_t i = (int64_t)blockIdx.x * NT + threadIdx.x; i < n; i += (int64_t)gridDim.x * NT) {
        double2 xv = x[i], yv = y[i];
// ... 493 lines not shown
            double2 v;
            if (VEC) {
                v = *reinterpret_cast<const double2 *>(p + k * stride);
            } else {
                v.x = p[k * stride];
                v.y = CPLX ? p[k * stride + 1] : 0.;
            }
            if (CPLX) {
                re0 = fma(c.x, v.x, re0);
                re0 = fma(-c.y, v.y, re0);
                im0 = fma(c.x, v.y, im0);
                im0 = fma(c.y, v.x, im0);
            } else {
                re0 = fma(c.x, v.x, re0);
                im0 = fma(c.y, v.x, im0);
                if (VEC) {
                    re1 = fma(c.x, v.y, re1);
                    im1 = fma(c.y, v.y, im1);
                }
            }
        }
        s = fma(re0, re0, s);
        s = fma(im0, im0, s);
        if (!CPLX && VEC) {
            s = fma(re1, re1, s);
            s = fma(im1, im1, s);
            reinterpret_cast<double2 *>(out)[2 * i] = double2{scale * re0, scale * im0};
            reinterpret_cast<double2 *>(out)[2 * i + 1] = double2{scale * re1, scale * im1};
        } else if (VEC) {
            reinterpret_cast<double2 *>(out)[i] = double2{scale * re0, scale * im0};
        } else {
            out[2 * i] = scale * re0;
            out[2 * i + 1] = scale * im0;
        }
    }
    s = block_sum<NT>(s, red);
    if (threadIdx.x == 0) {
        partial[2 * blockIdx.x] = s;
        partial[2 * blockIdx.x + 1] = 0.;
    }
}

__global__ void lz_post_scalars_kernel(const double *__restrict__ src, double *__restrict__ dst_host) {
    dst_host[0] = src[0];
    dst_host[1] = src[1];
    __threadfence_system();
}

__global__ __launch_bounds__(NT) void lz_copy_scaled_kernel(int64_t nd, const double *__restrict__ x, const double *__restrict__ nrm2,
                                                            double *__restrict__ y) {
    const double f = 1. / sqrt(nrm2[0]);
    for (int64_t i = (int64_t)blockIdx.x * NT + threadIdx.x; i < nd; i += (int64_t)gridDim.x * NT) y[i] = f * x[i];
}

struct LzHost {
    double *pinned = nullptr;
    int capacity = 0;
    std::vector<hipEvent_t> ev;
    std::vector<hipEvent_t> tev;
};
thread_local LzHost lz_host;

int lz_reserve(int steps) {
    LzHost &H = lz_host;
    if (H.capacity < steps + 2) {
        if (H.pinned) TPA_HIP_CHECK(hipHostFree(H.pinned));
        H.capacity = 2 * (steps + 2);
        TPA_HIP_CHECK(hipHostMalloc((void **)&H.pinned, sizeof(double) * 2 * H.capacity, hipHostMallocDefault));
    }
    while ((int)H.ev.size() < steps + 2) {
        hipEvent_t e;
        TPA_HIP_CHECK(hipEventCreateWithFlags(&e, hipEventDisableTiming));
        H.ev.push_back(e);
    }
    return 0;
}

inline void *lz_slot(int64_t s, void *const *bufs, int n_bufs, const void *in, void *out) {
    if (s == -1) return const_cast<void *>(in);
    if (s == -2) return out;
    return (s >= 0 && s < n_bufs) ? bufs[s] : nullptr;
}

}

static thread_local tpa_collective_callback lz_collective = nullptr;
static thread_local void *lz_collective_user = nullptr;
extern "C" int tpa_lanczos_set_collective(tpa_collective_callback cb, void *user) {
    lz_collective = cb;
    lz_collective_user = user;
    return 0;
}

static int lz_step_reortho(int dtype, int64_t n, double *w, const double *V, int k, double *ab_out, double *scratch, double *pw, void *stream) {
    hipStream_t st = (hipStream_t)stream;
    const bool cplx = (dtype == TPA_C128);
    const int64_t nd = cplx ? 2 * n : n;
    const double *vk = V + (int64_t)k * nd;
    const int g = grid_for(n, 8);
    double *part2 = scratch + 2 * MAXBLK;
    if (!cplx) {
        reduce_pass1<0><<<g, NT, 0, st>>>(n, w, vk, scratch);
        reduce_pass2<<<1, NT, 0, st>>>(g, scratch, ab_out);
        lanczos_update_dev_kernel<false, false><<<g, NT, 0, st>>>(n, w, ab_out, vk, nullptr, nullptr, part2);
    } else {
        reduce_pass1<1><<<g, NT, 0, st>>>(n, w, vk, scratch);
        reduce_pass2<<<1, NT, 0, st>>>(g, scratch, ab_out);
        lanczos_update_dev_kernel<true, false><<<g, NT, 0, st>>>(n, w, ab_out, vk, nullptr, nullptr, part2);
    }
    TPA_LAUNCH_CHECK();
    if (int rc = tpa_project_out(dtype, n, V, k, n, w, w, pw, ab_out + 1, pw + 2 * PJ_MAX + 2, stream)) return rc;
    scal_rsqrt_dev_kernel<<<grid_for(nd, 8), NT, 0, st>>>(nd, w, ab_out + 1);
    TPA_LAUNCH_CHECK();
    return 0;
}

extern "C" int tpa_lanczos_run(int dtype, int64_t n, const int64_t *ops, int n_ops, void *const *bufs, int n_bufs,
                               void *krylov_dev, const void *psi0_dev, int N_max, double cutoff, int has_shift, double E_shift,
                               double *scalars_dev, double *scratch_dev, tpa_lanczos_callback cb, void *user,
                               int time_gemms, double *info, void *stream) {
    return tpa_lanczos_run_ex(dtype, n, ops, n_ops, bufs, n_bufs, krylov_dev, psi0_dev, N_max, cutoff, has_shift, E_shift, scalars_dev,
                              scratch_dev, cb, user, time_gemms, info, 0, nullptr, stream);
}

extern "C" int tpa_lanczos_run_ex(int dtype, int64_t n, const int64_t *ops, int n_ops, void *const *bufs, int n_bufs,
                                  void *krylov_dev, const void *psi0_dev, int N_max, double cutoff, int has_shift, double E_shift,
                                  double *scalars_dev, double *scratch_dev, tpa_lanczos_callback cb, void *user,
                                  int time_gemms, double *info, int flags, double *project_work_dev, void *stream) {
    TPA_ARG_CHECK(dtype == TPA_F64 || dtype == TPA_C128);
    TPA_ARG_CHECK((flags & ~1) == 0 && (!(flags & 1) || (project_work_dev != nullptr && N_max <= PJ_MAX)));
    const bool reortho = (flags & 1) != 0;
    TPA_ARG_CHECK(n > 0 && N_max >= 1 && n_ops >= 1 && ops != nullptr && krylov_dev != nullptr && psi0_dev != nullptr);
    TPA_ARG_CHECK(scalars_dev != nullptr && scratch_dev != nullptr && cb != nullptr && info != nullptr);
    hipStream_t st = (hipStream_t)stream;
    const bool cplx = (dtype == TPA_C128);
    const int64_t nd = cplx ? 2 * n : n;
    double *V = (double *)krylov_dev;
    if (int rc = lz_reserve(N_max)) return rc;
    LzHost &H = lz_host;
    double *sc0 = scalars_dev + 2 * (N_max + 1);
    if (int rc = tpa_nrm2sq(dtype, n, psi0_dev, sc0, scratch_dev, stream)) return rc;
    lz_copy_scaled_kernel<<<grid_for(nd, 8), NT, 0, st>>>(nd, (const double *)psi0_dev, sc0, V);
    lz_post_scalars_kernel<<<1, 1, 0, st>>>(sc0, H.pinned + 2 * (N_max + 1));
    TPA_HIP_CHECK(hipEventRecord(H.ev[N_max + 1], st));
    size_t n_tev = 0;
    int n_matvec = 0, N = 0;
    bool stopped = false;
    for (int k = 0; k < N_max; ++k) {
        const double *vin = V + (int64_t)k * nd;
        double *w = V + (int64_t)(k + 1) * nd;
        for (int o = 0; o < n_ops; ++o) {
            const int64_t *op = ops + 12 * o;
            void *a = lz_slot(op[6], bufs, n_bufs, vin, w), *b = lz_slot(op[7], bufs, n_bufs, vin, w), *c = lz_slot(op[8], bufs, n_bufs, vin, w);
            if (op[0] == 0) {
                TPA_ARG_CHECK(a != nullptr && b != nullptr && c != nullptr);
                if (time_gemms) {
                    while (H.tev.size() < n_tev + 2) {
                        hipEvent_t e;
                        TPA_HIP_CHECK(hipEventCreate(&e));
                        H.tev.push_back(e);
                    }
                    TPA_HIP_CHECK(hipEventRecord(H.tev[n_tev], st));
                }
                if (int rc = tpa_gemm_chain(dtype, (int)op[1], (const int64_t *)op[2], (const int64_t *)op[3], (const int32_t *)op[4], (int)op[5],
                                            a, b, c, stream))
                    return rc;
                if (time_gemms) {
                    TPA_HIP_CHECK(hipEventRecord(H.tev[n_tev + 1], st));
                    n_tev += 2;
                }
            } else if (op[0] == 1) {
                TPA_ARG_CHECK(a != nullptr && c != nullptr);
                if (int rc = tpa_lincomb_batch(dtype, (const int64_t *)op[2], (int)op[5], (const int64_t *)op[3], op[9], a, c, stream)) return rc;
                if (time_gemms && op[1] == 1 && n_tev >= 2) TPA_HIP_CHECK(hipEventRecord(H.tev[n_tev - 1], st));
            } else if (op[0] == 2) {
                TPA_ARG_CHECK(a != nullptr && c != nullptr);
                if (int rc = tpa_copy_batch(dtype, (const int64_t *)op[2], (int)op[5], op[9], a, c, stream)) return rc;
            } else if (op[0] == 3) {
                TPA_ARG_CHECK(lz_collective != nullptr);
                if (int rc = lz_collective((int)op[1], lz_collective_user)) {
                    snprintf(tpa_errbuf, sizeof(tpa_errbuf), "tpa_lanczos_run: the collective callback of op %d failed (%d)", o, rc);
                    return TPA_E_BADARG;
                }
            } else if (op[0] == 4) {
                TPA_ARG_CHECK(a != nullptr && b != nullptr && c != nullptr && op[2] != 0 && op[5] >= 0 && op[5] <= PJ_MAX);
                double *pw = (double *)op[2];
                if (int rc = tpa_project_out(dtype, n, a, (int)op[5], op[3], b, c, pw, nullptr, pw + 2 * op[5] + 2, stream)) return rc;
            } else if (op[0] == 5) {
                TPA_ARG_CHECK(a != nullptr && c != nullptr);
                if (int rc = tpa_mpo_apply_batch(dtype, (const int64_t *)op[2], (int)op[5], (const int64_t *)op[3], (const void *)op[4],
                                                 (int)op[7], op[9], a, c, stream))
                    return rc;
            } else if (op[0] == 6) {
                TPA_ARG_CHECK(a != nullptr && c != nullptr);
                if (int rc = tpa_mpo_entry_apply_batch(dtype, (const int64_t *)op[2], (int)op[5], (const int64_t *)op[3], (const int64_t *)op[4],
                                                       op[9], a, c, stream))
                    return rc;
            } else {
                TPA_ARG_CHECK(false && "unknown op kind");
            }
        }
        ++n_matvec;
        if (has_shift)
            if (int rc = tpa_axpy(dtype, n, E_shift, 0., vin, w, stream)) return rc;
        if (reortho && k > 0) {
            if (int rc = lz_step_reortho(dtype, n, w, V, k, scalars_dev + 2 * k, scratch_dev, project_work_dev, stream)) return rc;
        } else if (int rc = tpa_lanczos_step(dtype, n, w, vin, k > 0 ? (const void *)(V + (int64_t)(k - 1) * nd) : nullptr,
                                             k > 0 ? scalars_dev + 2 * (k - 1) + 1 : nullptr, scalars_dev + 2 * k, scratch_dev, stream))
            return rc;
        lz_post_scalars_kernel<<<1, 1, 0, st>>>(scalars_dev + 2 * k, H.pinned + 2 * k);
        TPA_HIP_CHECK(hipEventRecord(H.ev[k], st));
        if (k == 0) {
            TPA_HIP_CHECK(hipEventSynchronize(H.ev[N_max + 1]));
            info[3] = sqrt(H.pinned[2 * (N_max + 1)]);
            if (!(info[3] >= cutoff)) {
                info[0] = 0.;
                info[1] = 1.;
                info[2] = 0.;
                TPA_HIP_CHECK(hipStreamSynchronize(st));
                return 0;
            }
        }
        if (k > 0) {
            TPA_HIP_CHECK(hipEventSynchronize(H.ev[k - 1]));
            if (cb(k - 1, H.pinned[2 * (k - 1)], H.pinned[2 * (k - 1) + 1], user)) {
                N = k;
                stopped = true;
                break;
            }
        }
        N = k + 1;
    }
    if (!stopped) {
        TPA_HIP_CHECK(hipEventSynchronize(H.ev[N_max - 1]));
        cb(N_max - 1, H.pinned[2 * (N_max - 1)], H.pinned[2 * (N_max - 1) + 1], user);
    }
    double ms = 0.;
    if (time_gemms && n_tev) {
        TPA_HIP_CHECK(hipEventSynchronize(H.tev[n_tev - 1]));
        for (size_t i = 0; i < n_tev; i += 2) {
            float t = 0.f;
            TPA_HIP_CHECK(hipEventElapsedTime(&t, H.tev[i], H.tev[i + 1]));
            ms += t;
        }
    }
    info[0] = (double)N;
    info[1] = (double)n_matvec;
    info[2] = ms;
    return 0;
}

extern "C" int tpa_krylov_combine(int dtype, int64_t n, const void *krylov_dev, int N, const double *coeff, void *out_dev,
                                  double *red_out_dev, double *scratch_dev, double *norm_host, void *stream) {
    TPA_ARG_CHECK(dtype == TPA_F64 || dtype == TPA_C128);
    TPA_ARG_CHECK(n > 0 && N >= 1 && N <= LZ_MAX_COMBINE && coeff != nullptr && out_dev != nullptr && norm_host != nullptr);
    hipStream_t st = (hipStream_t)stream;
    const bool cplx = (dtype == TPA_C128);
    const int64_t nd = cplx ? 2 * n : n;
    LzCoeff C;
    for (int k = 0; k < LZ_MAX_COMBINE; ++k) C.c[k] = k < N ? coeff[k] : 0.;
    const int g = grid_for(nd, 4);
    if (cplx)
        krylov_combine_kernel<true><<<g, NT, 0, st>>>(nd, N, C, (const double *)krylov_dev, nd, (double *)out_dev, scratch_dev);
    else
        krylov_combine_kernel<false><<<g, NT, 0, st>>>(nd, N, C, (const double *)krylov_dev, nd, (double *)out_dev, scratch_dev);
    reduce_pass2<<<1, NT, 0, st>>>(g, scratch_dev, red_out_dev);
    TPA_LAUNCH_CHECK();
    if (int rc = lz_reserve(1)) return rc;
    lz_post_scalars_kernel<<<1, 1, 0, st>>>(red_out_dev, lz_host.pinned);
    TPA_HIP_CHECK(hipEventRecord(lz_host.ev[0], st));
    TPA_HIP_CHECK(hipEventSynchronize(lz_host.ev[0]));
    norm_host[0] = sqrt(lz_host.pinned[0]);
    return 0;
}

extern "C" int tpa_krylov_combine_z(int basis_dtype, int64_t n, const void *krylov_dev, int N, const double *coeff, double scale,
                                    void *out_dev, double *red_out_dev, double *scratch_dev, double *norm_host, void *stream) {
    TPA_ARG_CHECK(basis_dtype == TPA_F64 || basis_dtype == TPA_C128);
    TPA_ARG_CHECK(n > 0 && N >= 1 && N <= LZ_MAX_COMBINE && krylov_dev != nullptr && coeff != nullptr && out_dev != nullptr);
    TPA_ARG_CHECK(red_out_dev != nullptr && scratch_dev != nullptr && norm_host != nullptr);
    hipStream_t st = (hipStream_t)stream;
    const bool cplx = (basis_dtype == TPA_C128);
    LzCoeffZ C;
    for (int k = 0; k < LZ_MAX_COMBINE; ++k) C.c[k] = k < N ? double2{coeff[2 * k], coeff[2 * k + 1]} : double2{0., 0.};
    const bool aligned = (((uintptr_t)krylov_dev | (uintptr_t)out_dev) & 15) == 0;
    const bool vec = aligned && (cplx || n % 2 == 0);
    const int64_t n_items = (!cplx && vec) ? n / 2 : n;
    const int64_t stride = cplx ? 2 * n : n;
    int64_t g64 = (n_items + NT - 1) / NT;
    const int g = (int)(g64 > 2 * MAXBLK ? 2 * MAXBLK : g64);
    const double *V = (const double *)krylov_dev;
    double *out = (double *)out_dev;
    if (cplx && vec)
        krylov_combine_z_kernel<true, true><<<g, NT, 0, st>>>(n_items, N, C, scale, V, stride, out, scratch_dev);
    else if (cplx)
        krylov_combine_z_kernel<true, false><<<g, NT, 0, st>>>(n_items, N, C, scale, V, stride, out, scratch_dev);
    else if (vec)
        krylov_combine_z_kernel<false, true><<<g, NT, 0, st>>>(n_items, N, C, scale, V, stride, out, scratch_dev);
    else
        krylov_combine_z_kernel<false, false><<<g, NT, 0, st>>>(n_items, N, C, scale, V, stride, out, scratch_dev);
    TPA_LAUNCH_CHECK();
    reduce_pass2<<<1, NT, 0, st>>>(g, scratch_dev, red_out_dev);
    TPA_LAUNCH_CHECK();
    if (int rc = lz_reserve(1)) return rc;
    lz_post_scalars_kernel<<<1, 1, 0, st>>>(red_out_dev, lz_host.pinned);
    TPA_HIP_CHECK(hipEventRecord(lz_host.ev[0], st));
    TPA_HIP_CHECK(hipEventSynchronize(lz_host.ev[0]));
    norm_host[0] = sqrt(lz_host.pinned[0]);
    return 0;
}
```

tenpy_amd/linalg/krylov_based.py:

```python
import logging

import numpy as np

from . import _device as dev
from . import np_conserved as npc

logger = logging.getLogger(__name__)

import os as _os
NATIVE = _os.environ.get('TPA_LANCZOS_NATIVE', '1') != '0'
PIPELINED = _os.environ.get('TPA_LANCZOS_PIPELINED', '1') != '0'

__all__ = ['LanczosGroundState', 'LanczosEvolution', 'Arnoldi', 'lanczos', 'gram_schmidt', 'iscale_prefactor', 'iadd_prefactor_other']


stats = {'runs': 0, 'n_matvec': 0, 'n_ill_conditioned': 0, 'n_degenerate': 0, 'n_native_sharded': 0, 'n_native_evolve': 0,
         'n_native_ortho': 0, 'n_ortho_declined': 0, 'n_native_reortho': 0}


class LanczosGroundState:

    def __init__(self, H, psi0, options):
        self.H = H
        self.psi0 = psi0.copy(deep=True)
        self.options = options = dict(options) if options is not None else {}
        self.N_min = int(options.get('N_min', 2))
        self.N_max = int(options.get('N_max', 20))
        self.P_tol = options.get('P_tol', 1.e-14)
        self.min_gap = options.get('min_gap', 1.e-12)
        self.reortho = bool(options.get('reortho', False))
        self.E_shift = options.get('E_shift', None)
        self.E_tol = options.get('E_tol', np.inf)
        self.N_cache = int(options.get('N_cache', self.N_max))
        if self.N_min < 2:
            raise ValueError("Should perform at least 2 steps.")
        if self.N_cache < 2:
            raise ValueError("Need to cache at least two vectors.")
        self._cutoff = options.get('cutoff', np.finfo(np.float64).eps * 100)
        self._cache = []
        self._psi0_norm = None
        self.Es = np.zeros([self.N_max, self.N_max], dtype=np.float64)
        self._h_krylov = np.zeros([self.N_max + 1, self.N_max + 1], dtype=np.float64)
        self._result_krylov = None

    def run(self):
        stats['runs'] += 1
        prog = self._native_program()
        if prog is not None:
            return self._run_native(prog)
        N = self._build_krylov()
        E0 = self.Es[N - 1, 0]
        if self.E_shift is not None:
            E0 -= self.E_shift
        if N == 1:
            return E0, self.psi0.copy(deep=True), N
        return E0, self._calc_result_full(N), N

    def _native_program(self):
        if not (NATIVE and PIPELINED) or self.N_cache < self.N_max or self.N_max + 1 > 64:
            return None
        make = getattr(self.H, 'native_input', None)
        if make is None:
            return None
        w = self.psi0
        if w.stored_blocks == 0 or not w._is_packed():
            return None
        got = make(w)
        if got is None:
            return None
        if self.reortho and len(got[1]) > 3:
            return None
        self.psi0, prog = got
        return prog

    def _run_native(self, prog):
        N, n, krylov, red = self._native_krylov(prog)
        L, w = dev.lib(), self.psi0
        code = dev.code(w.dtype)
        _, scr = dev.reduction_buffers()
        E0 = self.Es[N - 1, 0]
        if self.E_shift is not None:
            E0 -= self.E_shift
        psif = w.copy(deep=False)
        out = dev.empty(n, w.dtype)
        if N == 1:
            out.copy_(krylov[:n])
            psif._arena = out
            return E0, psif, N
        vf = np.ascontiguousarray(self._result_krylov, dtype=np.float64)
        assert len(vf) == N
        nrm = np.zeros(1, dtype=np.float64)
        dev.check(L.tpa_krylov_combine(code, n, krylov.data_ptr(), N, vf.ctypes.data, out.data_ptr(), red, scr.data_ptr(), nrm.ctypes.data,
                                       dev.stream()), "krylov_combine")
        nrm = float(nrm[0])
        psif._arena = out
        if abs(1. - nrm) > 1.e-5:
            stats['n_ill_conditioned'] += 1
            logger.warning("poorly conditioned H matrix in KrylovBased! |psi_0| = %f", nrm)
        if not (nrm > 1.e-8) or not np.isfinite(nrm):
            stats['n_degenerate'] += 1
            out.copy_(krylov[:n])
            nrm = 1.
        if nrm != 1.:
            dev.check(L.tpa_scal(code, n, 1. / nrm, 0., out.data_ptr(), dev.stream()), "scal")
        return E0, psif, N

    def _native_krylov(self, prog):
        from .. import _lib
        ops, bufs, gemm_plans = prog[:3]
        collective = prog[3] if len(prog) > 3 else None
        w = self.psi0
        n, dtype = w._arena.numel(), w.dtype
        code, L = dev.code(dtype), dev.lib()
        N_max = max(2, min(self.N_max, n))
        N_min_run = min(self.N_min, N_max)
        krylov = dev.scratch('lanczos_krylov', (N_max + 1) * n, dtype)
        scal = dev.scratch('lanczos_scalars', 2 * (N_max + 2) + 4, np.float64)
        _, scr = dev.reduction_buffers()
        h = self._h_krylov
        err = []

        def record(j, alpha, bsq, user):
            try:
                b = float(np.sqrt(bsq))
                h[j, j] = alpha
                if j + 2 >= N_min_run or j + 1 >= N_max or abs(b) < self._cutoff:
                    self._calc_result_krylov(j)
                h[j, j + 1] = h[j + 1, j] = b
                return int(abs(b) < self._cutoff or (j + 1 >= N_min_run and self._converged(j)))
            except BaseException as e:
                err.append(e)
                return 1
        cb = _lib.LANCZOS_CALLBACK(record)
        ptrs = np.array([t.data_ptr() for t in bufs], dtype=np.int64)
        info = np.zeros(4, dtype=np.float64)
        timed = npc.gemm_timer.sample()
        ccb = None
        if collective is not None:
            ccb = _lib.COLLECTIVE_CALLBACK(collective)
            L.tpa_lanczos_set_collective(ccb, None)
            stats['n_native_sharded'] = stats.get('n_native_sharded', 0) + 1
        failure = None
        flags = int(self.reortho)
        stats['n_native_reortho'] += flags
        extended = flags != 0 or bool(np.any(ops[:, 0] == 4))
        try:
            if not extended:
                dev.check(L.tpa_lanczos_run(code, n, ops.ctypes.data, len(ops), ptrs.ctypes.data, len(ptrs), krylov.data_ptr(),
                                            w._arena.data_ptr(), N_max, float(self._cutoff), int(self.E_shift is not None),
                                            float(self.E_shift or 0.), scal.data_ptr(), scr.data_ptr(), cb, None, int(timed),
                                            info.ctypes.data, dev.stream()), "lanczos_run")
            else:
                pw = dev.scratch('lanczos_project', 2 * _lib.PROJECT_MAX + 2 + _lib.PROJECT_WORK, np.float64) if flags else None
                dev.check(L.tpa_lanczos_run_ex(code, n, ops.ctypes.data, len(ops), ptrs.ctypes.data, len(ptrs), krylov.data_ptr(),
                                               w._arena.data_ptr(), N_max, float(self._cutoff), int(self.E_shift is not None),
                                               float(self.E_shift or 0.), scal.data_ptr(), scr.data_ptr(), cb, None, int(timed),
                                               info.ctypes.data, flags, pw.data_ptr() if flags else None, dev.stream()),
                          "lanczos_run_ex")
        except Exception as e:
            if collective is None:
                raise
            failure = e
        finally:
            if ccb is not None:
                L.tpa_lanczos_set_collective(_lib.COLLECTIVE_CALLBACK(), None)
        if err and failure is None:
            failure = err[0]
        agree = getattr(collective, 'agree', None)
        if agree is not None:
            if agree(failure is not None) and failure is None:
# ... 410 lines not shown
```

tenpy_amd/linalg/np_conserved.py:

```python
import functools
import threading
import warnings
from collections import OrderedDict

import os

import numpy as np
from hashlib import blake2b as _blake2b

from . import _device as dev
from .charges import QTYPE, ChargeInfo, DipolarChargeInfo, LegCharge, LegPipe, _find_row_differences, _partial_qtotal

__all__ = ['QCUTOFF', 'ChargeInfo', 'DipolarChargeInfo', 'LegCharge', 'LegPipe', 'Array', 'zeros', 'ones', 'eye_like', 'diag',
           'concatenate', 'grid_concat', 'grid_outer', 'detect_grid_outer_legcharge', 'detect_qtotal', 'detect_legcharge',
           'trace', 'outer', 'inner', 'tensordot', 'svd', 'pinv', 'norm', 'eigh', 'eig', 'eigvalsh', 'eigvals', 'speigs',
           'expm', 'qr', 'lq', 'polar', 'orthogonal_columns', 'to_iterable_arrays', 'TensordotPlan']

QCUTOFF = np.finfo(np.float64).eps * 10

COPY_MAXDIM = 6


@functools.lru_cache(maxsize=256)
def _calc_dtype(*dtypes):
# ... 1329 lines not shown
            cur = cur._project_axis(a, m, map_qind, new_leg)
        if cur is self or cur._arena is self._arena:
            cur = cur.copy(deep=True)
        keep_axes = [a for a in range(self.rank) if a not in axes]
        res = cur.copy(deep=False)
        res.legs = [cur.legs[a] for a in keep_axes]
        res._set_shape()
        res._labels = [self._labels[a] for a in keep_axes]
        res.qtotal = self.chinfo.make_valid(qtotal)
        res._qdata = np.ascontiguousarray(cur._qdata[:, keep_axes])
        res._skey = None
        return res

    def iunary_blockwise(self, func, *args, **kwargs):
        name = getattr(func, '__name__', None)
        name = {'conjugate': 'conj', 'absolute': 'abs'}.get(name, name)
        import torch as t
        f = getattr(t, name, None) if name else None
        if f is None or name not in _UNARY_OK:
            raise NotImplementedError("tenpy_amd: no device implementation of the element-wise function %r" % (func,))
        if self._arena is not None and self._arena.numel() > 0:
            if name == 'imag' and not self._arena.is_complex():
                out = t.zeros_like(self._arena)
            elif name == 'angle' and not self._arena.is_complex():
                out = t.angle(self._arena)
            else:
                out = f(self._arena, *args, **kwargs)
            if out.is_conj():
                out = out.resolve_conj()
            if out.dtype not in (t.float64, t.complex128):
                out = out.to(t.complex128 if out.is_complex() else t.float64)
            self._arena = out.contiguous()
            self.dtype = np.dtype(np.complex128 if out.is_complex() else np.float64)
        elif name in ('real', 'imag', 'abs', 'angle'):
            self.dtype = np.dtype(np.float64)
        self._skey = None
        return self

    def unary_blockwise(self, func, *args, **kwargs):
        res = self.copy(deep=True)
        return res.iunary_blockwise(func, *args, **kwargs)

    def matvec(self, other):
        return tensordot(self, other, axes=1)

    def gauge_total_charge(self, axis, newqtotal=None, new_qconj=None):
        res = self.copy(deep=False)
        ax = self.get_leg_index(axis)
        old = self.legs[ax]
        if new_qconj is None:
            new_qconj = old.qconj
        if new_qconj not in (-1, +1):
            raise ValueError("invalid new_qconj")
        res.qtotal = self.chinfo.make_valid(newqtotal).copy()
        shifted = old.charges + old.qconj * (res.qtotal - self.qtotal)
        if new_qconj != old.qconj:
            shifted = -shifted
        res.legs = list(self.legs)
        res.legs[ax] = LegCharge.from_qind(self.chinfo, old.slices, self.chinfo.make_valid(shifted), new_qconj)
        res._skey = None
        return res

    def add_trivial_leg(self, axis=0, label=None, qconj=1):
        if axis < 0:
            axis += self.rank + 1
        res = self.copy(deep=True)
        leg = LegCharge.from_trivial(1, self.chinfo, qconj)
        res.legs.insert(axis, leg)
        res._labels.insert(axis, label)
        res._set_shape()
        res._qdata = np.ascontiguousarray(np.insert(self._qdata, axis, 0, axis=1)).astype(np.intp)
        res._skey = None
        return res

    def add_leg(self, leg, i, axis=0, label=None):
        if axis < 0:
            axis += self.rank
        if label is not None and label in self._labels:
            raise ValueError("label already exists")
        qi, pos = leg.get_qindex(int(i) % leg.ind_len if -leg.ind_len <= i < leg.ind_len else int(i))
        width = int(leg.get_block_sizes()[qi])
        legs = list(self.legs)
        legs.insert(axis, leg)
        labels = list(self._labels)
        labels.insert(axis, label)
        res = Array(legs, self.dtype, self.chinfo.make_valid(self.qtotal + leg.get_charge(qi)), labels)
        qdata = np.ascontiguousarray(np.insert(self._qdata, axis, qi, axis=1)).astype(np.intp)
        if self.stored_blocks == 0:
            return res
        if width == 1:
            src = self.copy(deep=True)
            src._repack()
            res._set_blocks(qdata, arena=src._arena, qdata_sorted=False)
            return res
        res._set_blocks(qdata, zero=True, qdata_sorted=False)
        shapes = self._block_shapes()
        outer = np.prod(shapes[:, :axis], axis=1)
        inner = np.prod(shapes[:, axis:], axis=1)
        dst_off, src_off, sizes = [], [], []
        for b in range(self.stored_blocks):
            o = np.arange(outer[b], dtype=np.int64)
            dst_off.append(res._offsets[b] + (o * width + pos) * inner[b])
            src_off.append(self._offsets[b] + o * inner[b])
            sizes.append(np.full(outer[b], inner[b], dtype=np.int64))
        dst_off, src_off, sizes = np.concatenate(dst_off), np.concatenate(src_off), np.concatenate(sizes)
        _run_copy(self.dtype, _copy_jobs_contiguous(dst_off, src_off, sizes), int(np.max(sizes)), self._arena, res._arena)
        return res

    def squeeze(self, axes=None):
        if axes is None:
            axes = [a for a in range(self.rank) if self.shape[a] == 1]
        else:
            axes = self.get_leg_indices(_to_iterable(axes))
        for a in axes:
            if self.shape[a] != 1:
                raise ValueError("Tried to squeeze non-unit leg")
        keep = [a for a in range(self.rank) if a not in axes]
        if len(keep) == 0:
            v = self.to_ndarray()
            return v.reshape(-1)[0]
        res = self.copy(deep=True)
        res.legs = [self.legs[a] for a in keep]
        res._labels = [self._labels[a] for a in keep]
        res._set_shape()
        res._qdata = np.ascontiguousarray(self._qdata[:, keep])
        for a in axes:
            res.qtotal = res.qtotal - self.legs[a].get_charge(0)
        res.qtotal = self.chinfo.make_valid(res.qtotal)
        res._skey = None
        return res



_reshape_plans = OrderedDict()
_RESHAPE_PLANS_MAX = 16384


def clear_device_caches():
    _plan_cache.clear()
    _reshape_plans.clear()
    dev._pool.clear()
    if dev._table_cache is not None:
        dev._table_cache.clear()
        dev._table_bytes = 0
    _svd_warm._tables.clear()
    _svd_warm._plans.clear()
    _svd_warm.cache_clear()
    try:
        from ..algorithms import mps_common as _mc
        _mc._heff_plans.clear()
        _mc.MpoApplyPlan._cache.clear()
        _mc.MpoBlockApplyPlan._cache.clear()
        _mc.MpoEntryApplyPlan._cache.clear()
    except ImportError:
        pass


def _reshape_plan_get(key):
    pl = _reshape_plans.get(key)
    if pl is not None:
        try:
            _reshape_plans.move_to_end(key)
        except KeyError:
            pass
    return pl


def _reshape_plan_put(key, plan):
    for arr in plan[:2]:
        if isinstance(arr, np.ndarray):
            arr.setflags(write=False)
    _reshape_plans[key] = plan
    if len(_reshape_plans) > _RESHAPE_PLANS_MAX:
        _reshape_plans.popitem(last=False)


def _c_strides(shapes):
    shapes = np.asarray(shapes, dtype=np.int64)
    n, r = shapes.shape
    st = np.ones((n, r), dtype=np.int64)
    for a in range(r - 2, -1, -1):
        st[:, a] = st[:, a + 1] * shapes[:, a + 1]
    return st


def _copy_jobs_contiguous(dst_offs, src_offs, sizes):
    n = len(sizes)
    jobs = np.zeros((n, 4 + 3 * COPY_MAXDIM), dtype=np.int64)
    jobs[:, 0] = dst_offs
    jobs[:, 1] = src_offs
    jobs[:, 2] = 1
    jobs[:, 4] = sizes
    jobs[:, 4 + COPY_MAXDIM] = 1
    jobs[:, 4 + 2 * COPY_MAXDIM] = 1
    return jobs


def _run_copy(dtype, jobs, max_elems, src_arena, dst_arena):
    if len(jobs) == 0 or max_elems == 0:
        return
    L = dev.lib()
    for s in range(0, len(jobs), 60000):
        chunk = jobs[s:s + 60000]
        jd = dev.table(chunk)
        dev.check(L.tpa_copy_batch(dev.code(dtype), jd.data_ptr(), len(chunk), int(max_elems), src_arena.data_ptr(),
                                   dst_arena.data_ptr(), dev.stream()), "copy_batch")


def _scatter_blocks(src, layout, dst_arena):
    if src.stored_blocks == 0:
        return
    key = {tuple(r): i for i, r in enumerate(layout._qdata)}
    idx = np.array([key[tuple(r)] for r in src._qdata], dtype=np.int64)
    sizes = src._block_sizes_flat()
    jobs = _copy_jobs_contiguous(layout._offsets[idx], src._offsets, sizes)
    _run_copy(layout.dtype, jobs, int(np.max(sizes)), src._arena, dst_arena)



def zeros(legcharges, dtype=np.float64, qtotal=None, labels=None):
    return Array(legcharges, dtype, qtotal, labels)


def eye_like(a, axis=0, labels=None):
    return diag(1., a.get_leg(axis), labels=labels)


def diag(s, leg, dtype=None, labels=None):
    s = np.asarray(s, dtype)
    scalar = (s.ndim == 0)
    if not scalar and len(s) != leg.ind_len:
        raise ValueError("len(s)={0:d} not equal to leg.ind_len={1:d}".format(len(s), leg.ind_len))
    res = Array((leg, leg.conj()), s.dtype, labels=labels)
    qdata = np.arange(leg.block_number, dtype=np.intp)[:, np.newaxis] * np.ones(2, dtype=np.intp)[np.newaxis, :]
    blocks = []
    for q in range(leg.block_number):
        sl = leg.get_slice(q)
        d = np.full(sl.stop - sl.start, s) if scalar else s[sl]
        blocks.append(np.diag(d.astype(res.dtype)).reshape(-1))
    keep = [i for i, b in enumerate(blocks) if b.size]
    if keep:
        res._set_blocks(qdata[keep], arena=dev.to_device(np.concatenate([blocks[i] for i in keep])), qdata_sorted=True)
    return res


_UNARY_OK = {'conj', 'real', 'imag', 'abs', 'angle', 'sqrt', 'exp', 'log', 'square', 'negative', 'sign', 'sin', 'cos', 'tanh',
             'reciprocal'}


def ones(legcharges, dtype=np.float64, qtotal=None, labels=None):
    res = Array(legcharges, dtype, qtotal, labels)
    qdata = res._allowed_qdata()
    if len(qdata):
        res._set_blocks(qdata, qdata_sorted=True)
        res._arena.fill_(1.)
    return res


def concatenate(arrays, axis=0, copy=True):
    arrays = list(arrays)
    first = arrays[0]
    axis = first.get_leg_index(axis)
    not_axis = [a for a in range(first.rank) if a != axis]
    for a in arrays:
        if a.shape[:axis] != first.shape[:axis] or a.shape[axis + 1:] != first.shape[axis + 1:]:
            raise ValueError("wrong shape to fit " + repr(a.shape) + " into " + repr(first.shape))
        if a.chinfo != first.chinfo:
            raise ValueError("wrong ChargeInfo")
        if np.any(a.qtotal != first.qtotal):
            raise ValueError("wrong qtotal")
        for l in not_axis:
            a.legs[l].test_equal(first.legs[l])
    dtype = _calc_dtype(*[a.dtype for a in arrays])
    axis_qconj = first.legs[axis].qconj
    bl_sizes, charges, qdatas = [], [], []
    shift = 0
    for a in arrays:
        leg = a.legs[axis]
        bl_sizes.extend(leg.get_block_sizes())
        charges.append(leg.charges if leg.qconj == axis_qconj else first.chinfo.make_valid(-leg.charges))
        q = a._qdata.copy()
        q[:, axis] += shift
        qdatas.append(q)
        shift += leg.block_number
    legs = list(first.legs)
    legs[axis] = LegCharge.from_qind(first.chinfo, np.append([0], np.cumsum(bl_sizes)), np.concatenate(charges, axis=0), axis_qconj)
    res = Array(legs, dtype, first.qtotal, list(first._labels))
    res._set_blocks(np.concatenate(qdatas, axis=0), qdata_sorted=False)
    at = 0
    for a in arrays:
        if a.stored_blocks == 0:
            continue
        src = a if a.dtype == dtype else a.astype(dtype)
        sizes = src._block_sizes_flat()
        n = len(sizes)
        jobs = _copy_jobs_contiguous(res._offsets[at:at + n], src._offsets, sizes)
        _run_copy(dtype, jobs, int(np.max(sizes)), src._arena, res._arena)
        at += n
    return res


def expm(a):
    if a.rank != 2 or a.shape[0] != a.shape[1]:
        raise ValueError("expect a square matrix!")
    a.legs[0].test_contractible(a.legs[1])
    if np.any(a.qtotal != a.chinfo.make_valid()):
# ... 242 lines not shown
            break
        if n_res.value > cap_res or n_gemm.value > cap_gemm:
            cap_res, cap_gemm = max(cap_res, n_res.value), max(cap_gemm, n_gemm.value)
            continue
        _lib.check(rc, "plan_tensordot")
    nr, ng = n_res.value, n_gemm.value
    return res_q[:nr, :rr].reshape(nr, rr), gemm[:ng]


def _normalize_axes(a, b, axes):
    if isinstance(axes, (int, np.integer)):
        n = int(axes)
        axes_a = list(range(a.rank - n, a.rank))
        axes_b = list(range(n))
    else:
        axes_a, axes_b = axes
        axes_a = a.get_leg_indices(_to_iterable(axes_a))
        axes_b = b.get_leg_indices(_to_iterable(axes_b))
    if len(axes_a) != len(axes_b):
        raise ValueError("different lens of axes for a, b: " + repr(axes))
    if len(set(axes_a)) != len(axes_a) or len(set(axes_b)) != len(axes_b):
        raise ValueError("repeated axis")
    return axes_a, axes_b


def _matrix_form(rank, caxes):
    n = len(caxes)
    if n == 0:
        return 'trail'
    if list(caxes) == list(range(rank - n, rank)):
        return 'trail'
    if list(caxes) == list(range(n)):
        return 'lead'
    return None


def plan_tensordot(a, b, axes=2):
    axes_a, axes_b = _normalize_axes(a, b, axes)
    for la, lb in zip(axes_a, axes_b):
        a.legs[la].test_contractible(b.legs[lb])
    if a.chinfo != b.chinfo:
        raise ValueError("Different ChargeInfo")
    nc = len(axes_a)
    order = np.argsort(axes_a)
    ca = [axes_a[i] for i in order]
    cb = [axes_b[i] for i in order]
    fa = _matrix_form(a.rank, ca)
    a_use, b_use = a, b
    if fa is None:
        keep_a = [x for x in range(a.rank) if x not in axes_a]
        a_use = a.transpose(keep_a + list(axes_a))
        ca = list(range(a.rank - nc, a.rank))
        cb = list(axes_b)
        fa = 'trail'
    fb = _matrix_form(b.rank, cb)
    if fb is None:
        keep_b = [x for x in range(b.rank) if x not in cb]
        b_use = b.transpose(cb + keep_b)
        cb = list(range(nc))
        fb = 'lead'
    key = (a_use._struct_key(), b_use._struct_key(), tuple(ca), tuple(cb), a.dtype.str, b.dtype.str)
    plan = _plan_cache.get(key)
    if plan is not None:
        try:
            _plan_cache.move_to_end(key)
        except KeyError:
            pass
        return plan, a_use, b_use
    plan = _build_plan(a_use, b_use, ca, cb, fa, fb)
    _plan_cache[key] = plan
    if len(_plan_cache) > _PLAN_CACHE_SIZE:
        _plan_cache.popitem(last=False)
    return plan, a_use, b_use


def _build_plan(a, b, ca, cb, fa, fb):
    nc = len(ca)
    keep_a = [x for x in range(a.rank) if x not in ca]
    keep_b = [x for x in range(b.rank) if x not in cb]
    plan = TensordotPlan()
    plan.dtype = _calc_dtype(a.dtype, b.dtype)
    plan.keep_a, plan.keep_b = keep_a, keep_b
    if len(keep_a) + len(keep_b) == 0:
        raise ValueError("full contraction: use inner()")
    if a.stored_blocks == 0 or b.stored_blocks == 0:
        return plan
    aq = a._qdata[:, keep_a + list(ca)]
    bq = b._qdata[:, list(cb) + keep_b]
    contr_nblocks = [a.legs[x].block_number for x in ca]
    res_q, gemm = _plan_host(aq, bq, nc, contr_nblocks)
    if len(res_q) == 0:
        return plan
    plan.empty = False
    a_shapes, b_shapes = a._block_shapes(), b._block_shapes()
    M = np.prod(a_shapes[:, keep_a], axis=1).astype(np.int64) if keep_a else np.ones(a.stored_blocks, np.int64)
    K = np.prod(a_shapes[:, ca], axis=1).astype(np.int64) if nc else np.ones(a.stored_blocks, np.int64)
    N = np.prod(b_shapes[:, keep_b], axis=1).astype(np.int64) if keep_b else np.ones(b.stored_blocks, np.int64)
    nres = len(res_q)
    gi, ga, gb = gemm[:, 0], gemm[:, 1], gemm[:, 2]
    first = np.concatenate([[0], np.nonzero(np.diff(gi))[0] + 1])
    counts = np.diff(np.concatenate([first, [len(gi)]]))
    m_res, n_res = M[ga[first]], N[gb[first]]
    sizes = m_res * n_res
    offs = np.concatenate([[0], np.cumsum(sizes)])
    plan.res_qdata = np.ascontiguousarray(res_q, dtype=np.intp)
    plan.res_offsets = offs[:-1].astype(np.int64)
    plan.res_total = int(offs[-1])
    tmp = Array([a.legs[x] for x in keep_a] + [b.legs[x] for x in keep_b], plan.dtype)
    tmp._qdata, tmp._offsets = plan.res_qdata, plan.res_offsets
    plan.res_skey = tmp._struct_key()
    links = np.zeros((len(gi), 8), dtype=np.int64)
    links[:, 0] = a._offsets[ga]
    links[:, 1] = b._offsets[gb]
    links[:, 2] = K[ga]
    if fa == 'trail':
        links[:, 3], links[:, 4] = K[ga], 1
    else:
        links[:, 3], links[:, 4] = 1, M[ga]
    if fb == 'lead':
        links[:, 5], links[:, 6] = N[gb], 1
    else:
        links[:, 5], links[:, 6] = 1, K[ga]
    tasks = np.zeros((nres, 8), dtype=np.int64)
    tasks[:, 0] = plan.res_offsets
    tasks[:, 1], tasks[:, 2], tasks[:, 3] = m_res, n_res, n_res
    tasks[:, 4], tasks[:, 5] = first, counts
    ksum = np.add.reduceat(K[ga], first)
    pad = {}
    for cfg in (1, 0):
        bm, bn = _gemm_tile(plan.dtype, cfg)
        tm, tn = (m_res + bm - 1) // bm, (n_res + bn - 1) // bn
        ntile = tm * tn
        plan.cfg = cfg
        pad[cfg] = float(np.sum(ntile * ksum)) * bm * bn
    if FORCE_GEMM_CFG != 0 and (int(np.sum(ntile)) < GEMM_MIN_LARGE_TILES or (plan.dtype.kind != 'c' and pad[0] > GEMM_LARGE_TILE_PAD * pad[1])):
        plan.cfg = 1
        bm, bn = _gemm_tile(plan.dtype, 1)
        tm, tn = (m_res + bm - 1) // bm, (n_res + bn - 1) // bn
        ntile = tm * tn
    if FORCE_GEMM_CFG is not None and plan.cfg != FORCE_GEMM_CFG:
        plan.cfg = FORCE_GEMM_CFG
        bm, bn = _gemm_tile(plan.dtype, plan.cfg)
        tm, tn = (m_res + bm - 1) // bm, (n_res + bn - 1) // bn
        ntile = tm * tn
    t_task = np.repeat(np.arange(nres), ntile)
    local = np.arange(int(np.sum(ntile))) - np.repeat(np.cumsum(ntile) - ntile, ntile)
    t_row = local // np.repeat(tn, ntile)
    t_col = local % np.repeat(tn, ntile)
    work = np.repeat(ksum, ntile)
    order = _xcd_tile_order(t_task, t_row, t_col, work, np.repeat(tm, ntile), np.repeat(tn, ntile))
    tiles = np.zeros((len(t_task), 4), dtype=np.int32)
    tiles[:, 0], tiles[:, 1], tiles[:, 2] = t_task[order], t_row[order], t_col[order]
    plan.n_tiles = len(tiles)
    plan.tasks_host, plan.links_host = tasks, links
    plan.tasks_dev, plan.links_dev, plan.tiles_dev = dev.to_device_packed(tasks, links, tiles)
    cmul = 8 if plan.dtype.kind == 'c' else 2
    plan.flops = int(cmul * np.sum(M[ga] * K[ga] * N[gb]))
    esz = 16 if plan.dtype.kind == 'c' else 8
    ua, ub = np.unique(ga), np.unique(gb)
    plan.bytes_min = int(esz * (np.sum(M[ua] * K[ua]) + np.sum(K_of_b(b_shapes, cb, ub) * N[ub]) + plan.res_total))
    plan.n_gemm = len(gi)
    plan.gemm_shapes = np.stack([M[ga], K[ga], N[gb]], axis=1)
    plan.sk = _split_k(plan, tasks, links, tm, tn)
    return plan


GEMM_SPLIT_K = tuple(int(x) for x in os.environ.get('TPA_GEMM_SPLIT_K', '4,4096,128,1024').split(','))
GEMM_K_TILE = 16


class _SplitK:
    __slots__ = ('tasks_dev', 'links_dev', 'tiles_dev', 'n_tiles', 'total', 'jobs_dev', 'terms_dev', 'n_jobs', 'max_elems',
                 'tasks_host', 'links_host', 'jobs_host', 'terms_host', 'parts')


def _split_k(plan, tasks, links, tm, tn, knob=None):
    knob = tuple(knob or GEMM_SPLIT_K)
    s_max, target, min_k, max_tiles = knob + (4096, 128, 1024)[len(knob) - 1:]
    if s_max < 2 or plan.n_tiles * 2 > target or plan.n_tiles > max_tiles or len(tasks) > 65535:
        return None
    s_plan = min(s_max, target // plan.n_tiles)
    nt = len(tasks)
    first, counts = tasks[:, 4], tasks[:, 5]
    assert np.array_equal(first, np.cumsum(counts) - counts) and first[-1] + counts[-1] == len(links)
    K = links[:, 2]
    g_end = np.cumsum(K)
    g_start = g_end - K
    t_start, t_end = g_start[first], g_end[first + counts - 1]
    ktot = t_end - t_start
    s_t = np.clip(ktot // max(min_k, 1), 1, s_plan)
    if np.all(s_t == 1):
        return None
    n_cut = s_t - 1
    ct = np.repeat(np.arange(nt), n_cut)
    cj = np.arange(int(np.sum(n_cut))) - np.repeat(np.cumsum(n_cut) - n_cut, n_cut) + 1
    pos = t_start[ct] + ktot[ct] * cj // s_t[ct]
    li = np.searchsorted(g_start, pos, side='right') - 1
    pos = g_start[li] + np.minimum((pos - g_start[li] + GEMM_K_TILE // 2) // GEMM_K_TILE * GEMM_K_TILE, K[li])
    bt = np.concatenate([np.arange(nt), ct, np.arange(nt)])
    bp = np.concatenate([t_start, pos, t_end])
    order = np.lexsort((bp, bt))
    bt, bp = bt[order], bp[order]
    keep = (bt[:-1] == bt[1:]) & (bp[1:] > bp[:-1])
    p_task, p0, p1 = bt[:-1][keep], bp[:-1][keep], bp[1:][keep]
    n_new = len(p_task)
    if n_new == nt:
        return None
    l0 = np.searchsorted(g_start, p0, side='right') - 1
    l1 = np.searchsorted(g_start, p1, side='left')
    nl = l1 - l0
    lb = np.cumsum(nl) - nl
    idx = np.repeat(l0, nl) + np.arange(int(np.sum(nl))) - np.repeat(lb, nl)
    new_links = links[idx].copy()
    c0 = np.maximum(np.repeat(p0, nl), g_start[idx]) - g_start[idx]
    c1 = np.minimum(np.repeat(p1, nl), g_end[idx]) - g_start[idx]
    new_links[:, 0] += c0 * new_links[:, 4]
    new_links[:, 1] += c0 * new_links[:, 5]
    new_links[:, 2] = c1 - c0
    m, n = tasks[p_task, 1], tasks[p_task, 2]
    offs = np.cumsum(m * n) - m * n
    new_tasks = np.zeros((n_new, 8), dtype=np.int64)
    new_tasks[:, 0], new_tasks[:, 1], new_tasks[:, 2], new_tasks[:, 3], new_tasks[:, 4], new_tasks[:, 5] = offs, m, n, n, lb, nl
    terms = np.zeros((n_new, 4), dtype=np.int64)
    terms[:, 0], terms[:, 1], terms[:, 2] = offs, n, np.array(1.0).view(np.int64)
    parts = np.bincount(p_task, minlength=nt)
    jobs = np.zeros((nt, 8), dtype=np.int64)
    jobs[:, :4] = tasks[:, :4]
    jobs[:, 4], jobs[:, 5] = np.cumsum(parts) - parts, parts
    works = p1 - p0
    off = int(np.sum(m * n))
    sk = _SplitK()
    sk.parts = parts
    ntile = np.repeat(tm * tn, sk.parts)
    t_task = np.repeat(np.arange(n_new), ntile)
    local = np.arange(int(np.sum(ntile))) - np.repeat(np.cumsum(ntile) - ntile, ntile)
    tn_new, tm_new = np.repeat(tn, sk.parts), np.repeat(tm, sk.parts)
    t_row, t_col = local // np.repeat(tn_new, ntile), local % np.repeat(tn_new, ntile)
    order = _xcd_tile_order(t_task, t_row, t_col, np.repeat(works, ntile), np.repeat(tm_new, ntile),
                            np.repeat(tn_new, ntile))
    tiles = np.zeros((len(t_task), 4), dtype=np.int32)
    tiles[:, 0], tiles[:, 1], tiles[:, 2] = t_task[order], t_row[order], t_col[order]
    sk.tasks_host, sk.links_host, sk.jobs_host, sk.terms_host = new_tasks, new_links, jobs, terms
    sk.tasks_dev, sk.links_dev, sk.tiles_dev, sk.jobs_dev, sk.terms_dev = dev.to_device_packed(sk.tasks_host, sk.links_host, tiles, sk.jobs_host,
                                                                                            sk.terms_host)
    sk.n_tiles, sk.total, sk.n_jobs = len(tiles), off, len(jobs)
    sk.max_elems = int(np.max(tasks[:, 1] * tasks[:, 2]))
    return sk


N_XCD = 8
XCD_TILE_ORDER = True


def _xcd_tile_order(t_task, t_row, t_col, work, tm, tn):
    n = len(t_task)
    if not XCD_TILE_ORDER or n < 2 * N_XCD:
        return np.argsort(-work, kind='stable')
    xcd = np.where(tm >= N_XCD, (t_row * N_XCD) // np.maximum(tm, 1),
                   ((t_row * tn + t_col) * N_XCD) // np.maximum(tm * tn, 1)).astype(np.int64)
    xcd = (xcd + t_task) % N_XCD
    key = np.lexsort((t_col, t_row, t_task, -work, xcd))
    lists = [key[xcd[key] == x] for x in range(N_XCD)]
    target = -(-n // N_XCD)
    spill = []
    for x in range(N_XCD):
        if len(lists[x]) > target:
            spill.extend(lists[x][target:])
            lists[x] = lists[x][:target]
    for x in range(N_XCD):
        need = target - len(lists[x])
        if need > 0 and spill:
            lists[x] = np.concatenate([lists[x], np.array(spill[:need], dtype=np.int64)])
            spill = spill[need:]
    out = np.full(target * N_XCD, -1, dtype=np.int64)
    for x in range(N_XCD):
        out[x:x + N_XCD * len(lists[x]):N_XCD] = lists[x]
    out = out[out >= 0]
    assert len(out) == n
    return out


def K_of_b(b_shapes, cb, idx):
    return np.prod(b_shapes[idx][:, cb], axis=1) if len(cb) else np.ones(len(idx), np.int64)


def tensordot(a, b, axes=2):
    axes_a, axes_b = _normalize_axes(a, b, axes)
    if len(axes_a) == a.rank and len(axes_b) == b.rank:
        return inner(a, b, axes=(axes_a, axes_b), do_conj=False)
    plan, a_use, b_use = plan_tensordot(a, b, (axes_a, axes_b))
    return plan.apply(a_use, b_use)


def outer(a, b):
    return tensordot(a, b, axes=0)


def inner(a, b, axes='labels', do_conj=False):
    if isinstance(a, list) and isinstance(b, list):
        return np.sum([inner(w, v, axes=axes, do_conj=do_conj) for w, v in zip(a, b)])
    if a.rank != b.rank:
        raise ValueError("different rank!")
    if not (isinstance(axes, str) and axes == 'range'):
        if isinstance(axes, str) and axes == 'labels':
            a_labels = a.get_leg_labels()
            axes = (a_labels, a_labels) if do_conj else (a_labels, [Array._conj_leg_label(l) for l in a_labels])
        axes_a, axes_b = axes
        axes_a = a.get_leg_indices(_to_iterable(axes_a))
        axes_b = b.get_leg_indices(_to_iterable(axes_b))
        if len(axes_a) != a.rank or len(axes_b) != b.rank:
            raise ValueError("no full contraction. Use tensordot instead!")
        order = np.argsort(axes_b)
        axes_a = [axes_a[i] for i in order]
        if tuple(axes_a) != tuple(range(a.rank)):
            a = a.transpose(axes_a)
    if a.chinfo != b.chinfo:
        raise ValueError("different ChargeInfo")
    for lega, legb in zip(a.legs, b.legs):
        if do_conj:
            lega.test_equal(legb)
        else:
            lega.test_contractible(legb)
    if do_conj:
        if np.any(a.qtotal != b.qtotal):
            return _calc_dtype(a.dtype, b.dtype).type(0)
    else:
        if np.any(a.chinfo.make_valid(a.qtotal + b.qtotal) != 0):
            return _calc_dtype(a.dtype, b.dtype).type(0)
    calc = _calc_dtype(a.dtype, b.dtype)
    if a.stored_blocks == 0 or b.stored_blocks == 0:
        return calc.type(0)
    if a.dtype != calc:
        a = a.astype(calc)
    if b.dtype != calc:
        b = b.astype(calc)
    out, scr = dev.reduction_buffers()
    L = dev.lib()
    if a._same_structure(b) and a._is_packed():
        xa, xb, n = a._arena, b._arena, a._arena.numel()
    else:
        keyb = {tuple(r): i for i, r in enumerate(b._qdata)}
        ia = [i for i, r in enumerate(a._qdata) if tuple(r) in keyb]
        if len(ia) == 0:
            return calc.type(0)
        ib = [keyb[tuple(a._qdata[i])] for i in ia]
        sizes = a._block_sizes_flat()[ia]
        offs = np.concatenate([[0], np.cumsum(sizes)[:-1]]).astype(np.int64)
        n = int(np.sum(sizes))
        xa, xb = dev.empty(n, calc), dev.empty(n, calc)
        _run_copy(calc, _copy_jobs_contiguous(offs, a._offsets[ia], sizes), int(np.max(sizes)), a._arena, xa)
        _run_copy(calc, _copy_jobs_contiguous(offs, b._offsets[ib], sizes), int(np.max(sizes)), b._arena, xb)
    dev.check(L.tpa_dot(dev.code(calc), n, xa.data_ptr(), xb.data_ptr(), int(bool(do_conj)), out.data_ptr(),
                        scr.data_ptr(), dev.stream()), "dot")
    val = dev.read_scalar(out, calc.kind == 'c')
    return calc.type(val)


def norm(a, ord=None, convert_to_float=True):
    if isinstance(a, Array):
        return a.norm(ord, convert_to_float)
    return np.linalg.norm(np.asarray(a).reshape(-1), ord)


def trace(a, leg1=0, leg2=1):
    ax1, ax2 = a.get_leg_indices([leg1, leg2])
    a.legs[ax1].test_contractible(a.legs[ax2])
    eye = diag(1., a.legs[ax2], dtype=a.dtype)
    if a.rank == 2:
        return inner(a, eye, axes=([ax1, ax2], [0, 1]), do_conj=False)
    return tensordot(a, eye, axes=([ax1, ax2], [0, 1]))



SVD_ABS_FLOOR = float(os.environ.get('TPA_SVD_ABS_FLOOR', '1e-2'))
SVD_FLOOR_ON_MIN = os.environ.get('TPA_SVD_FLOOR_ON_MIN', '1') != '0'


def _svd_tol_arg():
    f = _svd_floor_now[0]
    return -f if (SVD_FLOOR_ON_MIN and f > 0.) else f
SVD_ABS_FLOOR_GENERIC = float(os.environ.get('TENPY_AMD_SVD_FLOOR', '0'))
svd_engine_floor = False


class _PerThreadFloor(threading.local):

    def __init__(self):
        self.v = SVD_ABS_FLOOR_GENERIC

    def __getitem__(self, i):
        return self.v

    def __setitem__(self, i, value):
        self.v = value

# ... 1141 lines not shown
```

Measured before the change: 1.852.

## Fold single-term MPO apply into second GEMM via scaled A2 links and skip unused tiles

Adds an extended GEMM chain kernel whose links can read from a second A buffer with a per-link scalar coefficient. In the two-site effective Hamiltonian matvec, MPO-apply jobs that have a single term are folded into the final GEMM's links, so they read straight from the first GEMM's output scaled by alpha. First-stage tiles whose output is never used are dropped. The aim is to remove the intermediate MPO-apply copy pass and wasted tile work in each Lanczos matvec, at the cost of host-side table construction, an extra FMA in staging, and new code paths limited to real f64 data.

After: 1.773, median of 6. 4.3% less time.

```diff
diff --git a/include/tenpy_amd.h b/include/tenpy_amd.h
--- a/include/tenpy_amd.h
+++ b/include/tenpy_amd.h
@@ -21,6 +21,12 @@
 int tpa_gemm_chain(int dtype, int cfg, const int64_t *tasks_dev, const int64_t *links_dev,
                    const int32_t *tiles_dev, int n_tiles, const void *Abase, const void *Bbase,
                    void *Cbase, void *stream);
+int tpa_gemm_chain_ex(int dtype, int cfg, const int64_t *tasks_dev, const int64_t *links_dev, const int32_t *tiles_dev, int n_tiles,
+                      const void *Abase, const void *A2base, const void *Bbase, void *Cbase, const double *alphas_dev, void *stream);
+
+int tpa_gemm_kernel_id(int dtype, int cfg, int n_tiles);
+
+int tpa_unit_defect_batch(int dtype, const int64_t *jobs_dev, int n_jobs, const void *src_base, double *out_dev, void *stream);
 
 int tpa_herk_tile_shape(int dtype, int *bt);
 int tpa_herk_chain(int dtype, const int64_t *tasks_dev, const int64_t *links_dev, const int32_t *tiles_dev, int n_tiles,
diff --git a/tenpy_amd/_lib.py b/tenpy_amd/_lib.py
--- a/tenpy_amd/_lib.py
+++ b/tenpy_amd/_lib.py
@@ -24,6 +24,9 @@
     "tpa_gemm_tile_shape": (ctypes.c_int, [ctypes.c_int, ctypes.c_int, ctypes.POINTER(ctypes.c_int), ctypes.POINTER(ctypes.c_int)]),
     "tpa_gemm_set_variant": (ctypes.c_int, [ctypes.c_int]),
     "tpa_gemm_chain": (ctypes.c_int, [ctypes.c_int, ctypes.c_int, _vp, _vp, _vp, ctypes.c_int, _vp, _vp, _vp, _vp]),
+    "tpa_gemm_chain_ex": (ctypes.c_int, [ctypes.c_int, ctypes.c_int, _vp, _vp, _vp, ctypes.c_int, _vp, _vp, _vp, _vp, _vp, _vp]),
+    "tpa_gemm_kernel_id": (ctypes.c_int, [ctypes.c_int, ctypes.c_int, ctypes.c_int]),
+    "tpa_unit_defect_batch": (ctypes.c_int, [ctypes.c_int, _vp, ctypes.c_int, _vp, _vp, _vp]),
     "tpa_herk_tile_shape": (ctypes.c_int, [ctypes.c_int, ctypes.POINTER(ctypes.c_int)]),
     "tpa_herk_chain": (ctypes.c_int, [ctypes.c_int, _vp, _vp, _vp, ctypes.c_int, _vp, _vp, _vp, _vp, _vp]),
     "tpa_axpy": (ctypes.c_int, [ctypes.c_int, ctypes.c_int64, ctypes.c_double, ctypes.c_double, _vp, _vp, _vp]),
diff --git a/tenpy_amd/algorithms/mps_common.py b/tenpy_amd/algorithms/mps_common.py
--- a/tenpy_amd/algorithms/mps_common.py
+++ b/tenpy_amd/algorithms/mps_common.py
@@ -13,6 +13,7 @@
 BLOCK_APPLY = _os.environ.get('TPA_MPO_BLOCK_APPLY', '1') != '0'
 from .._lib import MPO_APPLY_MAXD
 ENTRY_APPLY = int(_os.environ.get('TPA_MPO_ENTRY_APPLY', '1'))
+MATVEC_SKIP = _os.environ.get('TPA_MATVEC_UNIT', '1') != '0'
 
 def _env_set_LP(env, i, LP):
     if hasattr(env, 'get_LP_age'):
@@ -114,6 +115,7 @@
 
 from collections import OrderedDict as _OrderedDict
 _heff_plans = _OrderedDict()
+_skip_table_cache = _OrderedDict()
 
 
 def _fused_heff(env_t, W, left):
@@ -714,6 +716,7 @@
         _share_mpo_tables(self.W0, W0)
         _share_mpo_tables(self.W1, W1)
         self._env = env
+        self._skip_ok = tensors is None and not getattr(env.H, 'explicit_plus_hc', False)
         self._LHeff = self._RHeff = None
         self._plans = None
         self._fplans = None
@@ -869,6 +872,9 @@
             ok = (p1.dtype == a01.dtype == p2.dtype == theta.dtype == self._LPf.dtype == self._RPf.dtype and not p1.empty and
                   not p2.empty and not a01.empty)
             if ok:
+                res = self._skip_program(theta, fp)
+                last = p2
+            if ok and res is None:
                 bufs = [self._LPf._arena, self._RPf._arena, dev.scratch('lanczos_t1', p1.res_total, p1.dtype),
                         dev.scratch('lanczos_t3', a01.total, a01.dtype)]
                 ops = _gemm_ops(p1, 0, -1, 2, bufs, 'lanczos_sk1')
@@ -899,6 +905,134 @@
 
     def _plan_matches(self, theta):
         return self._plans[2] == theta._struct_key() and self._plans[3] == theta.dtype
+
+    def _skip_program(self, theta, fp):
+        from ..linalg import krylov_based as kb
+        p1, a01, p2 = fp['p1'], fp['a01'], fp['p2']
+        if not MATVEC_SKIP or not (p2.res_total == theta._arena.numel() and np.array_equal(p2.res_qdata, theta._qdata) and
+                                   np.array_equal(p2.res_offsets, theta._offsets)):
+            return None
+
+        def declined(reason):
+            kb.stats['n_skip_declined'] += 1
+            kb.skip_declined[reason] = kb.skip_declined.get(reason, 0) + 1
+            return None
+        if type(self) is not TwoSiteH or not self._skip_ok:
+            return declined('operator')
+        if type(a01) is not MpoApplyPlan:
+            return declined('mpo_plan')
+        if theta.dtype != np.float64:
+            return declined('dtype')
+        if not (dev.lib_provides('tpa_gemm_chain_ex') and hasattr(dev.lib(), 'tpa_gemm_kernel_id')):
+            return declined('library')
+        key = (id(p1), id(a01), id(p2))
+        hit = _skip_table_cache.get(key)
+        if hit is not None and hit[0] is p1 and hit[1] is a01 and hit[2] is p2:
+            _skip_table_cache.move_to_end(key)
+            et = hit[3]
+        else:
+            et = self._skip_tables(fp)
+            _skip_table_cache[key] = (p1, a01, p2, et)
+            if len(_skip_table_cache) > 1024:
+                _skip_table_cache.popitem(last=False)
+        if isinstance(et, str):
+            return declined(et)
+        kb.stats['n_skip_taken'] += 1
+        bufs = [self._LPf._arena, self._RPf._arena, dev.scratch('lanczos_t1', p1.res_total, p1.dtype),
+                dev.scratch('lanczos_t3', a01.total, a01.dtype)]
+        if et['a_tiles'] is None:
+            ops = _gemm_ops(p1, 0, -1, 2, bufs, 'lanczos_sk1')
+        elif p1.sk is None:
+            ops = [[0, p1.cfg, p1.tasks_dev.data_ptr(), p1.links_dev.data_ptr(), et['a_tiles'].data_ptr(), len(et['a_tiles']), 0, -1, 2, 0, 0, 0]]
+        else:
+            sk = p1.sk
+            bufs.append(dev.scratch('lanczos_sk1', sk.total, p1.dtype))
+            ops = [[0, p1.cfg, sk.tasks_dev.data_ptr(), sk.links_dev.data_ptr(), et['a_tiles'].data_ptr(), len(et['a_tiles']), 0, -1,
+                    len(bufs) - 1, 0, 0, 0],
+                   [1, 1, et['a_jobs'].data_ptr(), sk.terms_dev.data_ptr(), 0, len(et['a_jobs']), len(bufs) - 1, 0, 2, sk.max_elems, 0, 0]]
+        if et['b_jobs'] is not None:
+            ops.append([1, 0, et['b_jobs'].data_ptr(), a01.terms_dev.data_ptr(), 0, len(et['b_jobs']), 2, 0, 3, a01.max_elems, 0, 0])
+        sk = p2.sk
+        if sk is None:
+            ops.append([7, p2.cfg, p2.tasks_dev.data_ptr(), et['c_links'].data_ptr(), p2.tiles_dev.data_ptr(), p2.n_tiles, 3, 1, -2, 2,
+                        et['alphas'].data_ptr(), 0])
+        else:
+            bufs.append(dev.scratch('lanczos_sk2', sk.total, p2.dtype))
+            part = len(bufs) - 1
+            ops.append([7, p2.cfg, sk.tasks_dev.data_ptr(), et['c_links'].data_ptr(), sk.tiles_dev.data_ptr(), sk.n_tiles, 3, 1, part, 2,
+                        et['alphas'].data_ptr(), 0])
+            ops.append([1, 1, sk.jobs_dev.data_ptr(), sk.terms_dev.data_ptr(), 0, sk.n_jobs, part, 0, -2, sk.max_elems, 0, 0])
+        self.flops_per_matvec = et['plan_a'].flops + p2.flops
+        self.bytes_per_matvec = et['plan_a'].bytes_min + p2.bytes_min + et['b_bytes']
+        self.gemm_shapes = (et['plan_a'].gemm_shapes, p2.gemm_shapes)
+        return (np.array(ops, dtype=np.int64), bufs, (et['plan_a'], p2))
+
+    @staticmethod
+    def _skip_tables(fp):
+        p1, a01, p2 = fp['p1'], fp['a01'], fp['p2']
+        jobs3, terms3 = a01.jobs_host, a01.terms_host
+        t1_off = np.asarray(p1.res_offsets, dtype=np.int64)
+        term_t1 = np.searchsorted(t1_off, terms3[:, 0])
+        if not np.array_equal(t1_off[np.minimum(term_t1, len(t1_off) - 1)], terms3[:, 0]):
+            return 'term_inside_block'
+        order = np.argsort(jobs3[:, 0])
+        j_off, j_size = jobs3[order, 0], jobs3[order, 1] * jobs3[order, 2]
+        single, first_term = jobs3[order, 5] == 1, jobs3[order, 4]
+        links = (p2.links_host if p2.sk is None else p2.sk.links_host).copy()
+        lj = np.clip(np.searchsorted(j_off, links[:, 0], side='right') - 1, 0, len(j_off) - 1)
+        inside = (links[:, 0] >= j_off[lj]) & (links[:, 0] < j_off[lj] + j_size[lj])
+        if not np.all(inside | (links[:, 2] <= 0)):
+            return 'link_outside_blocks'
+        swap = inside & single[lj] & (links[:, 2] > 0)
+        term = first_term[lj[swap]]
+        if np.any(terms3[term, 1] != j_size[lj[swap]]):
+            return 'term_shape'
+        alpha = terms3[:, 2:4].copy().view(np.float64)[:, 0]
+        ualpha, ai = np.unique(alpha[term], return_inverse=True)
+        if len(ualpha) + 1 > 0xffff:
+            return 'too_many_coefficients'
+        alphas = np.zeros(2 * (len(ualpha) + 1), dtype=np.float64)
+        alphas[0], alphas[2::2] = 1., ualpha
+        links[swap, 0] = terms3[term, 0] + (links[swap, 0] - j_off[lj[swap]])
+        links[swap, 7] = (links[swap, 7] & 3) | 4 | ((ai.reshape(-1) + 1) << 16)
+        multi = np.sort(order[~single])
+        et = dict(a_tiles=None, a_jobs=None, b_jobs=None)
+        b_elems = 0
+        if len(multi):
+            in_multi = np.zeros(len(terms3), dtype=bool)
+            starts, counts = jobs3[multi, 4], jobs3[multi, 5]
+            in_multi[np.repeat(starts, counts) + np.arange(int(np.sum(counts))) - np.repeat(np.cumsum(counts) - counts, counts)] = True
+            b_elems = int(np.sum(terms3[in_multi, 1]) + np.sum(jobs3[multi, 1] * jobs3[multi, 2]))
+        need = np.zeros(len(t1_off), dtype=bool)
+        need[term_t1] = True
+        plan_a = p1
+        if not np.all(need):
+            sk, t1 = p1.sk, p1.tasks_host
+            src = p1.tiles_host if sk is None else sk.tiles_host
+            tile_task = src[:, 0] if sk is None else np.repeat(np.arange(len(t1_off)), sk.parts)[src[:, 0]]
+            kept = np.ascontiguousarray(src[need[tile_task]])
+            kernel = dev.lib().tpa_gemm_kernel_id
+            if kernel(dev.code(p1.dtype), p1.cfg, len(kept)) == kernel(dev.code(p1.dtype), p1.cfg, len(src)):
+                cnt = t1[need, 5]
+                lk = np.repeat(t1[need, 4], cnt) + np.arange(int(np.sum(cnt))) - np.repeat(np.cumsum(cnt) - cnt, cnt)
+                mt, nt_, kk = np.repeat(t1[need, 1], cnt), np.repeat(t1[need, 2], cnt), p1.links_host[lk, 2]
+                _, ua = np.unique(p1.links_host[lk, 0], return_index=True)
+                _, ub = np.unique(p1.links_host[lk, 1], return_index=True)
+                from types import SimpleNamespace
+                plan_a = SimpleNamespace(flops=int(2 * np.sum(mt * kk * nt_)), gemm_shapes=np.stack([mt, kk, nt_], axis=1),
+                                         bytes_min=int(8 * (np.sum(mt[ua] * kk[ua]) + np.sum(kk[ub] * nt_[ub]) + np.sum(t1[need, 1] * t1[need, 2]))))
+                if sk is None:
+                    (et['a_tiles'],) = dev.to_device_packed(kept)
+                else:
+                    et['a_tiles'], et['a_jobs'] = dev.to_device_packed(kept, np.ascontiguousarray(sk.jobs_host[need]))
+        if et['a_tiles'] is None and not np.any(swap):
+            return 'nothing_to_skip'
+        if len(multi):
+            et['c_links'], et['alphas'], et['b_jobs'] = dev.to_device_packed(links, alphas, np.ascontiguousarray(jobs3[multi]))
+        else:
+            et['c_links'], et['alphas'] = dev.to_device_packed(links, alphas)
+        et['plan_a'], et['b_bytes'], et['n_swapped'] = plan_a, 8 * b_elems, int(np.sum(swap))
+        return et
 
     def update_LP(self, env, i, U=None):
         assert i == self.i0 + 1
diff --git a/tenpy_amd/csrc/tpa_gemm.hip b/tenpy_amd/csrc/tpa_gemm.hip
--- a/tenpy_amd/csrc/tpa_gemm.hip
+++ b/tenpy_amd/csrc/tpa_gemm.hip
@@ -10,6 +10,32 @@
 struct Task {
     int64_t c_off, m, n, ldc, link_begin, link_count, accumulate, pad;
 };
+
+constexpr int64_t LINK_A2 = 4, LINK_UNIT = 8;
+__device__ __forceinline__ double link_alpha(const Link &L, const double *__restrict__ alphas) {
+    const int ia = (int)((L.flags >> 16) & 0xffff);
+    return ia ? alphas[2 * ia] : 1.0;
+}
+template <int TM, int TN>
+__device__ __forceinline__ void add_unit_links(d4 (&acc)[TM][TN], const Link *__restrict__ lk, const int nl, const double *__restrict__ Abase,
+                                               const double *__restrict__ A2base, const double *__restrict__ alphas, const int row_base,
+                                               const int col_base, const int m, const int n) {
+    for (int l = 0; l < nl; ++l) {
+        const Link L = lk[l];
+        if (!(L.flags & LINK_UNIT)) continue;
+        const double al = link_alpha(L, alphas);
+        const double *src = ((L.flags & LINK_A2) ? A2base : Abase) + L.a_off;
+#pragma unroll
+        for (int i = 0; i < TM; ++i)
+#pragma unroll
+            for (int j = 0; j < TN; ++j)
+#pragma unroll
+                for (int r = 0; r < 4; ++r) {
+                    const int row = row_base + i * 16 + 4 * r, col = col_base + j * 16;
+                    if (row < m && col < n) acc[i][j][r] = fma(al, src[(int64_t)row * L.a_rs + (int64_t)col * L.a_ks], acc[i][j][r]);
+                }
+    }
+}
 
 template <int ES, int NT, int BM, int BN>
 __device__ __forceinline__ bool gemm_identity_rows_tile(const Task &tk, const Link *__restrict__ links, const int4 tile, const double *__restrict__ Bbase,
@@ -53,10 +79,12 @@
     int i0, istep, lim;
 };
 
-template <bool CPLX, int BM, int BN, int TM, int TN, int BK_>
+template <bool CPLX, int BM, int BN, int TM, int TN, int BK_, bool EX = false>
 __global__ __launch_bounds__((Cfg<CPLX, BM, BN, TM, TN, BK_>::NT)) void gemm_chain_kernel(
     const Task *__restrict__ tasks, const Link *__restrict__ links, const int4 *__restrict__ tiles,
-    const double *__restrict__ Abase, const double *__restrict__ Bbase, double *__restrict__ Cbase) {
+    const double *__restrict__ Abase, const double *__restrict__ Bbase, double *__restrict__ Cbase,
+    const double *__restrict__ A2base, const double *__restrict__ alphas) {
+    static_assert(!(EX && CPLX), "extended links: real data only");
     using C = Cfg<CPLX, BM, BN, TM, TN, BK_>;
     constexpr int NT = C::NT, EA = C::EA, EB = C::EB, PL = C::PLANES, BK = C::BK;
     constexpr int ES = CPLX ? 2 : 1;
@@ -88,6 +116,7 @@
         Stage a, b;
         int K, sa_i, sa_k, sb_j, sb_k;
         double sgn_a, sgn_b;
+        double al;
         int64_t oa[EA], ob[EB];
     };
     auto open_link = [&](int li, LinkView &v) {
@@ -97,6 +126,8 @@
         const bool b_kfast = (L.b_ks == 1) && (L.b_ns != 1);
         v.sgn_a = (CPLX && (L.flags & 1)) ? -1.0 : 1.0;
         v.sgn_b = (CPLX && (L.flags & 2)) ? -1.0 : 1.0;
+        const double *Asrc = (EX && (L.flags & LINK_A2)) ? A2base : Abase;
+        if (EX) v.al = link_alpha(L, alphas);
         v.sa_i = a_kfast ? (BK + 1) : 1;
         v.sa_k = a_kfast ? 1 : (BM + C::PADA);
         v.sb_j = b_kfast ? (BK + 1) : 1;
@@ -104,7 +135,7 @@
         {
             const int i = a_kfast ? (tid / BK) : (tid % BM), kk = a_kfast ? (tid % BK) : (tid / BM);
             const int di = a_kfast ? (NT / BK) : 0, dk = a_kfast ? 0 : (NT / BM);
-            v.a.p = Abase + ES * (L.a_off + (int64_t)(row0 + i) * L.a_rs + (int64_t)kk * L.a_ks);
+            v.a.p = Asrc + ES * (L.a_off + (int64_t)(row0 + i) * L.a_rs + (int64_t)kk * L.a_ks);
             v.a.gstep = ES * ((int64_t)di * L.a_rs + (int64_t)dk * L.a_ks);
             v.a.kstep = ES * (int64_t)BK * L.a_ks;
             v.a.lbase = i * v.sa_i + kk * v.sa_k;
@@ -170,7 +201,7 @@
 #pragma unroll
         for (int r = 0; r < EA; ++r)
 #pragma unroll
-            for (int p = 0; p < PL; ++p) Ad[p * C::A_LDS + v.a.lbase + r * v.a.lstep] = ra[p][r];
+            for (int p = 0; p < PL; ++p) Ad[p * C::A_LDS + v.a.lbase + r * v.a.lstep] = EX ? fma(v.al, ra[p][r], 0.0) : ra[p][r];
 #pragma unroll
         for (int r = 0; r < EB; ++r)
 #pragma unroll
@@ -233,6 +264,8 @@
         }
     }
 
+    if constexpr (EX) add_unit_links<TM, TN>(acc[0], lk, nl, Abase, A2base, alphas, row0 + wr * TM * 16 + l4, col0 + wc * TN * 16 + l15, m, n);
+
     double *Cp = Cbase + ES * tk.c_off;
     const bool accum = tk.accumulate != 0;
 #pragma unroll
@@ -274,11 +307,12 @@
     static_assert(NT % BK == 0 && NT % BM == 0 && NT % BN == 0, "staging offsets must be affine in the element index");
 };
 
-template <int BM, int BN, int TM, int TN>
+template <int BM, int BN, int TM, int TN, bool EX = false>
 __global__ __launch_bounds__((Cfg2<BM, BN, TM, TN>::NT)) __attribute__((amdgpu_waves_per_eu(TM * TN >= 16 ? 2 : (TM * TN >= 8 ? 3 : 4))))
 void gemm_chain2_kernel(
     const Task *__restrict__ tasks, const Link *__restrict__ links, const int4 *__restrict__ tiles,
-    const double *__restrict__ Abase, const double *__restrict__ Bbase, double *__restrict__ Cbase) {
+    const double *__restrict__ Abase, const double *__restrict__ Bbase, double *__restrict__ Cbase,
+    const double *__restrict__ A2base, const double *__restrict__ alphas) {
     using C = Cfg2<BM, BN, TM, TN>;
     constexpr int NT = C::NT, EA = C::EA, EB = C::EB, BK = C::BK, LD = C::LD, IMG = C::IMG;
     extern __shared__ double lds2[];
@@ -309,16 +343,18 @@
         int kka, dka, kkb, dkb;
         int la, dla, lb, dlb;
         int K;
+        double al;
     };
     auto open_link = [&](int li, View &v) {
         const Link L = lk[li];
         v.K = (int)L.k;
+        if (EX) v.al = link_alpha(L, alphas);
         const bool a_kfast = (L.a_ks == 1);
         const bool b_kfast = (L.b_ks == 1) && (L.b_ns != 1);
         {
             const int i = a_kfast ? (tid / BK) : (tid % BM), kk = a_kfast ? (tid % BK) : (tid / BM);
             const int di = a_kfast ? (NT / BK) : 0, dk = a_kfast ? 0 : (NT / BM);
-            v.pa = Abase + L.a_off;
+            v.pa = ((EX && (L.flags & LINK_A2)) ? A2base : Abase) + L.a_off;
             v.ka = (int64_t)BK * L.a_ks;
             v.kka = kk;
             v.dka = dk;
@@ -360,7 +396,7 @@
     };
     auto store_tile = [&](const View &v, double *img) {
 #pragma unroll
-        for (int r = 0; r < EA; ++r) img[v.la + r * v.dla] = ra[r];
+        for (int r = 0; r < EA; ++r) img[v.la + r * v.dla] = EX ? fma(v.al, ra[r], 0.0) : ra[r];
 #pragma unroll
         for (int r = 0; r < EB; ++r) img[C::A_LDS + v.lb + r * v.dlb] = rb[r];
     };
@@ -428,6 +464,8 @@
         }
     }
 
+    if constexpr (EX) add_unit_links<TM, TN>(acc, lk, nl, Abase, A2base, alphas, row0 + wr * TM * 16 + l4, col0 + wc * TN * 16 + l15, m, n);
+
     double *Cp = Cbase + tk.c_off;
     const bool accum = tk.accumulate != 0;
 #pragma unroll
@@ -463,28 +501,36 @@
     return 0;
 }
 
-template <bool CPLX, int BM, int BN, int TM, int TN, int BK_>
+extern "C" int tpa_gemm_kernel_id(int dtype, int cfg, int n_tiles) {
+    if (dtype != TPA_F64) return 0;
+    if (cfg == 0) return 1;
+    return (n_tiles <= 1024 && !(g_variant & 1)) ? 0 : 1;
+}
+
+template <bool CPLX, int BM, int BN, int TM, int TN, int BK_, bool EX = false>
 static void launch(const int64_t *tasks_dev, const int64_t *links_dev, const int32_t *tiles_dev, int n_tiles,
-                   const void *Abase, const void *Bbase, void *Cbase, hipStream_t st) {
+                   const void *Abase, const void *Bbase, void *Cbase, hipStream_t st, const void *A2base = nullptr,
+                   const double *alphas = nullptr) {
     using C = Cfg<CPLX, BM, BN, TM, TN, BK_>;
-    gemm_chain_kernel<CPLX, BM, BN, TM, TN, BK_><<<n_tiles, C::NT, 0, st>>>(
+    gemm_chain_kernel<CPLX, BM, BN, TM, TN, BK_, EX><<<n_tiles, C::NT, 0, st>>>(
         (const Task *)tasks_dev, (const Link *)links_dev, (const int4 *)tiles_dev, (const double *)Abase,
-        (const double *)Bbase, (double *)Cbase);
-}
-
-template <int BM, int BN, int TM, int TN>
+        (const double *)Bbase, (double *)Cbase, (const double *)A2base, alphas);
+}
+
+template <int BM, int BN, int TM, int TN, bool EX = false>
 static int launch2(const int64_t *tasks_dev, const int64_t *links_dev, const int32_t *tiles_dev, int n_tiles,
-                   const void *Abase, const void *Bbase, void *Cbase, hipStream_t st) {
+                   const void *Abase, const void *Bbase, void *Cbase, hipStream_t st, const void *A2base = nullptr,
+                   const double *alphas = nullptr) {
     using C = Cfg2<BM, BN, TM, TN>;
     static bool attr_set = false;
     if (!attr_set) {
-        TPA_HIP_CHECK(hipFuncSetAttribute((const void *)gemm_chain2_kernel<BM, BN, TM, TN>, hipFuncAttributeMaxDynamicSharedMemorySize,
+        TPA_HIP_CHECK(hipFuncSetAttribute((const void *)gemm_chain2_kernel<BM, BN, TM, TN, EX>, hipFuncAttributeMaxDynamicSharedMemorySize,
                                           C::LDS_BYTES));
         attr_set = true;
     }
-    gemm_chain2_kernel<BM, BN, TM, TN><<<n_tiles, C::NT, C::LDS_BYTES, st>>>(
+    gemm_chain2_kernel<BM, BN, TM, TN, EX><<<n_tiles, C::NT, C::LDS_BYTES, st>>>(
         (const Task *)tasks_dev, (const Link *)links_dev, (const int4 *)tiles_dev, (const double *)Abase,
-        (const double *)Bbase, (double *)Cbase);
+        (const double *)Bbase, (double *)Cbase, (const double *)A2base, alphas);
     return 0;
 }
 
@@ -499,7 +545,7 @@
     if (dtype == TPA_F64) {
         if (cfg == 0)
             rc = launch2<128, 64, 4, 2>(tasks_dev, links_dev, tiles_dev, n_tiles, Abase, Bbase, Cbase, st);
-        else if (n_tiles <= 1024 && !(g_variant & 1))
+        else if (tpa_gemm_kernel_id(dtype, cfg, n_tiles) == 0)
             launch<false, 64, 64, 1, 2, 16>(tasks_dev, links_dev, tiles_dev, n_tiles, Abase, Bbase, Cbase, st);
         else
             rc = launch2<64, 64, 2, 2>(tasks_dev, links_dev, tiles_dev, n_tiles, Abase, Bbase, Cbase, st);
@@ -513,3 +559,23 @@
     TPA_LAUNCH_CHECK();
     return 0;
 }
+
+extern "C" int tpa_gemm_chain_ex(int dtype, int cfg, const int64_t *tasks_dev, const int64_t *links_dev, const int32_t *tiles_dev,
+                                 int n_tiles, const void *Abase, const void *A2base, const void *Bbase, void *Cbase,
+                                 const double *alphas_dev, void *stream) {
+    TPA_ARG_CHECK(dtype == TPA_F64);
+    TPA_ARG_CHECK(cfg == 0 || cfg == 1);
+    TPA_ARG_CHECK(A2base != nullptr && alphas_dev != nullptr);
+    if (n_tiles <= 0) return 0;
+    hipStream_t st = (hipStream_t)stream;
+    int rc = 0;
+    if (cfg == 0)
+        rc = launch2<128, 64, 4, 2, true>(tasks_dev, links_dev, tiles_dev, n_tiles, Abase, Bbase, Cbase, st, A2base, alphas_dev);
+    else if (tpa_gemm_kernel_id(dtype, cfg, n_tiles) == 0)
+        launch<false, 64, 64, 1, 2, 16, true>(tasks_dev, links_dev, tiles_dev, n_tiles, Abase, Bbase, Cbase, st, A2base, alphas_dev);
+    else
+        rc = launch2<64, 64, 2, 2, true>(tasks_dev, links_dev, tiles_dev, n_tiles, Abase, Bbase, Cbase, st, A2base, alphas_dev);
+    if (rc) return rc;
+    TPA_LAUNCH_CHECK();
+    return 0;
+}
diff --git a/tenpy_amd/csrc/tpa_util.hip b/tenpy_amd/csrc/tpa_util.hip
--- a/tenpy_amd/csrc/tpa_util.hip
+++ b/tenpy_amd/csrc/tpa_util.hip
@@ -14,3 +14,48 @@
     if (hbm_bytes) *hbm_bytes = (int64_t)p.totalGlobalMem;
     return 0;
 }
+
+namespace {
+constexpr int UD_NT = 256;
+struct UnitJob {
+    int64_t off, n, ld, pad;
+};
+
+template <bool CPLX>
+__global__ __launch_bounds__(UD_NT) void unit_defect_kernel(const UnitJob *__restrict__ jobs, const double *__restrict__ src,
+                                                            unsigned long long *__restrict__ out) {
+    const UnitJob J = jobs[blockIdx.y];
+    const int64_t total = J.n * J.n;
+    double worst = 0.0;
+    for (int64_t e = (int64_t)blockIdx.x * UD_NT + threadIdx.x; e < total; e += (int64_t)gridDim.x * UD_NT) {
+        const int64_t r = e / J.n, c = e - r * J.n;
+        const int64_t g = J.off + r * J.ld + c;
+        const double one = (r == c) ? 1.0 : 0.0;
+        double d;
+        if (CPLX)
+            d = hypot(src[2 * g] - one, src[2 * g + 1]);
+        else
+            d = fabs(src[g] - one);
+        if (!(d == d)) d = __builtin_huge_val();
+        worst = fmax(worst, d);
+    }
+    worst = wave_max(worst);
+    if ((threadIdx.x & 63) == 0 && worst > 0.0) atomicMax(out, (unsigned long long)__double_as_longlong(worst));
+}
+}
+
+extern "C" int tpa_unit_defect_batch(int dtype, const int64_t *jobs_dev, int n_jobs, const void *src_base, double *out_dev, void *stream) {
+    TPA_ARG_CHECK(dtype == TPA_F64 || dtype == TPA_C128);
+    TPA_ARG_CHECK(n_jobs >= 0 && n_jobs <= 65535 && out_dev != nullptr);
+    hipStream_t st = (hipStream_t)stream;
+    TPA_HIP_CHECK(hipMemsetAsync(out_dev, 0, sizeof(double), st));
+    if (n_jobs == 0) return 0;
+    TPA_ARG_CHECK(jobs_dev != nullptr && src_base != nullptr);
+    const dim3 grid(16, n_jobs);
+    if (dtype == TPA_F64)
+        unit_defect_kernel<false><<<grid, UD_NT, 0, st>>>((const UnitJob *)jobs_dev, (const double *)src_base, (unsigned long long *)out_dev);
+    else
+        unit_defect_kernel<true><<<grid, UD_NT, 0, st>>>((const UnitJob *)jobs_dev, (const double *)src_base, (unsigned long long *)out_dev);
+    TPA_LAUNCH_CHECK();
+    return 0;
+}
diff --git a/tenpy_amd/csrc/tpa_vec.hip b/tenpy_amd/csrc/tpa_vec.hip
--- a/tenpy_amd/csrc/tpa_vec.hip
+++ b/tenpy_amd/csrc/tpa_vec.hip
@@ -669,8 +669,10 @@
         for (int o = 0; o < n_ops; ++o) {
             const int64_t *op = ops + 12 * o;
             void *a = lz_slot(op[6], bufs, n_bufs, vin, w), *b = lz_slot(op[7], bufs, n_bufs, vin, w), *c = lz_slot(op[8], bufs, n_bufs, vin, w);
-            if (op[0] == 0) {
+            if (op[0] == 0 || op[0] == 7) {
                 TPA_ARG_CHECK(a != nullptr && b != nullptr && c != nullptr);
+                const void *a2 = op[0] == 7 ? lz_slot(op[9], bufs, n_bufs, vin, w) : nullptr;
+                TPA_ARG_CHECK(op[0] == 0 || (a2 != nullptr && op[10] != 0));
                 if (time_gemms) {
                     while (H.tev.size() < n_tev + 2) {
                         hipEvent_t e;
@@ -679,8 +681,10 @@
                     }
                     TPA_HIP_CHECK(hipEventRecord(H.tev[n_tev], st));
                 }
-                if (int rc = tpa_gemm_chain(dtype, (int)op[1], (const int64_t *)op[2], (const int64_t *)op[3], (const int32_t *)op[4], (int)op[5],
-                                            a, b, c, stream))
+                if (int rc = op[0] == 0 ? tpa_gemm_chain(dtype, (int)op[1], (const int64_t *)op[2], (const int64_t *)op[3],
+                                                         (const int32_t *)op[4], (int)op[5], a, b, c, stream)
+                                        : tpa_gemm_chain_ex(dtype, (int)op[1], (const int64_t *)op[2], (const int64_t *)op[3],
+                                                            (const int32_t *)op[4], (int)op[5], a, a2, b, c, (const double *)op[10], stream))
                     return rc;
                 if (time_gemms) {
                     TPA_HIP_CHECK(hipEventRecord(H.tev[n_tev + 1], st));
diff --git a/tenpy_amd/linalg/krylov_based.py b/tenpy_amd/linalg/krylov_based.py
--- a/tenpy_amd/linalg/krylov_based.py
+++ b/tenpy_amd/linalg/krylov_based.py
@@ -15,7 +15,9 @@
 
 
 stats = {'runs': 0, 'n_matvec': 0, 'n_ill_conditioned': 0, 'n_degenerate': 0, 'n_native_sharded': 0, 'n_native_evolve': 0,
-         'n_native_ortho': 0, 'n_ortho_declined': 0, 'n_native_reortho': 0}
+         'n_native_ortho': 0, 'n_ortho_declined': 0, 'n_native_reortho': 0,
+         'n_skip_taken': 0, 'n_skip_declined': 0}
+skip_declined = {}
 
 
 class LanczosGroundState:
diff --git a/tenpy_amd/linalg/np_conserved.py b/tenpy_amd/linalg/np_conserved.py
--- a/tenpy_amd/linalg/np_conserved.py
+++ b/tenpy_amd/linalg/np_conserved.py
@@ -1505,6 +1505,7 @@
         _mc.MpoApplyPlan._cache.clear()
         _mc.MpoBlockApplyPlan._cache.clear()
         _mc.MpoEntryApplyPlan._cache.clear()
+        _mc._skip_table_cache.clear()
     except ImportError:
         pass
 
@@ -2053,7 +2054,7 @@
     tiles = np.zeros((len(t_task), 4), dtype=np.int32)
     tiles[:, 0], tiles[:, 1], tiles[:, 2] = t_task[order], t_row[order], t_col[order]
     plan.n_tiles = len(tiles)
-    plan.tasks_host, plan.links_host = tasks, links
+    plan.tasks_host, plan.links_host, plan.tiles_host = tasks, links, tiles
     plan.tasks_dev, plan.links_dev, plan.tiles_dev = dev.to_device_packed(tasks, links, tiles)
     cmul = 8 if plan.dtype.kind == 'c' else 2
     plan.flops = int(cmul * np.sum(M[ga] * K[ga] * N[gb]))
@@ -2072,7 +2073,7 @@
 
 class _SplitK:
     __slots__ = ('tasks_dev', 'links_dev', 'tiles_dev', 'n_tiles', 'total', 'jobs_dev', 'terms_dev', 'n_jobs', 'max_elems',
-                 'tasks_host', 'links_host', 'jobs_host', 'terms_host', 'parts')
+                 'tasks_host', 'links_host', 'jobs_host', 'terms_host', 'parts', 'tiles_host')
 
 
 def _split_k(plan, tasks, links, tm, tn, knob=None):
@@ -2141,7 +2142,7 @@
                             np.repeat(tn_new, ntile))
     tiles = np.zeros((len(t_task), 4), dtype=np.int32)
     tiles[:, 0], tiles[:, 1], tiles[:, 2] = t_task[order], t_row[order], t_col[order]
-    sk.tasks_host, sk.links_host, sk.jobs_host, sk.terms_host = new_tasks, new_links, jobs, terms
+    sk.tasks_host, sk.links_host, sk.jobs_host, sk.terms_host, sk.tiles_host = new_tasks, new_links, jobs, terms, tiles
     sk.tasks_dev, sk.links_dev, sk.tiles_dev, sk.jobs_dev, sk.terms_dev = dev.to_device_packed(sk.tasks_host, sk.links_host, tiles, sk.jobs_host,
                                                                                             sk.terms_host)
     sk.n_tiles, sk.total, sk.n_jobs = len(tiles), off, len(jobs)
```
